# cr1m5onk1ng/text_similarity

Hardware: AMD Instinct MI355X
Metric: sentences/sec encoded + Mpairs/sec cosine top-k @ N=1M d=384 (higher is better)
Workload: dtype bf16 encoder / f16 selection / fp32 scores

## Files before the change

text_similarity_amd/csrc/encoder.hip:

```cpp
#include <math.h>
#include <cmath>

#include <stdlib.h>
#include <string.h>

#include <vector>

#include <type_traits>
#include <utility>

#include "common.h"
#include "gemm_pp.h"

namespace tsim {

__device__ __forceinline__ int64_t packed_off(int64_t t, int f, int W) {
    return ((t >> 5) * (W >> 3) + (f >> 3)) * 256 + (t & 31) * 8 + (f & 7);
}

template <int VPL, bool TYPED = false>
__global__ __launch_bounds__(256) void embed_ln_kernel(const int32_t *__restrict__ ids,
                                                       const int32_t *__restrict__ pos,
                                                       const float *__restrict__ word,
                                                       const float *__restrict__ pos_emb,
                                                       const float *__restrict__ type_tab,
                                                       const float *__restrict__ gamma,
                                                       const float *__restrict__ beta, float eps, int T, int H,
                                                       bf16_t *__restrict__ out, int vocab, int max_pos,
                                                       const int32_t *__restrict__ col, int max_len,
                                                       int *__restrict__ err_flags,
                                                       const int32_t *__restrict__ tok_type = nullptr, int n_types = 0) {
    const int lane = threadIdx.x & 63;
    const int t = blockIdx.x * 4 + (threadIdx.x >> 6);
    if (t >= T) return;
    int id = ids[t], ps = pos[t];
    int ty = 0;
    if constexpr (TYPED) ty = tok_type[t];
    int bad = 0;
    if (id < 0 || id >= vocab) { bad |= TSIM_ENC_ERR_TOKEN_ID; id = id < 0 ? 0 : vocab - 1; }
    if (ps < 0 || ps >= max_pos) { bad |= TSIM_ENC_ERR_POSITION; ps = ps < 0 ? 0 : max_pos - 1; }
    if (col[t] >= max_len || col[t] < 0) bad |= TSIM_ENC_ERR_MAX_LEN;
    if constexpr (TYPED) {
        if (ty < 0 || ty >= n_types) { bad |= TSIM_ENC_ERR_TOKEN_TYPE; ty = ty < 0 ? 0 : n_types - 1; }
    }
    if (bad && lane == 0) atomicOr(err_flags, bad);
    const float *w = word + (int64_t)id * H;
    const float *p = pos_emb + (int64_t)ps * H;
    const float *type_row = TYPED ? type_tab + (int64_t)ty * H : type_tab;
    float v[VPL], pv[VPL], tv[VPL];
#pragma unroll
    for (int i = 0; i < VPL; ++i) {
        v[i] = w[lane + i * 64];
        pv[i] = p[lane + i * 64];
    }
    if (type_row) {
#pragma unroll
        for (int i = 0; i < VPL; ++i) tv[i] = type_row[lane + i * 64];
    }
    float s = 0.f;
#pragma unroll
    for (int i = 0; i < VPL; ++i) {
        float a = v[i];
        if (type_row) a += tv[i];
        a += pv[i];
        v[i] = a;
        s += a;
    }
    const float mean = wave_sum(s) / (float)H;
    float q = 0.f;
#pragma unroll
    for (int i = 0; i < VPL; ++i) {
        const float dlt = v[i] - mean;
        q = fmaf(dlt, dlt, q);
    }
    const float rstd = 1.0f / sqrtf(wave_sum(q) / (float)H + eps);
#pragma unroll
    for (int i = 0; i < VPL; ++i) {
        const int j = lane + i * 64;
        out[(int64_t)t * H + j] = f32_to_bf16((v[i] - mean) * rstd * gamma[j] + beta[j]);
    }
}

enum { EPI_BIAS = 0, EPI_GELU = 1, EPI_RES_LN = 2 };

template <int BM, int BN, int BK, int WAVES_M, int WAVES_N, int NST = 2>
constexpr int gemm_lds_bytes() {
    return NST * (BM + BN) * BK * 2;
}

template <int BM, int BN, int BK, int WAVES_M, int WAVES_N, int EPI, int NST = 2>
__global__ __launch_bounds__(WAVES_M *WAVES_N * 64) void gemm_bf16_kernel(
    const bf16_t *__restrict__ X, const bf16_t *__restrict__ W, const float *__restrict__ bias,
    const bf16_t *__restrict__ res, const float *__restrict__ gamma, const float *__restrict__ beta, float eps,
    bf16_t *__restrict__ out, int M, int N, int K, int mtiles, int ntiles, const bf16_t *__restrict__ Wimg, int xpacked) {
    constexpr int NW = WAVES_M * WAVES_N;
    constexpr int TM = BM / WAVES_M, TN = BN / WAVES_N, MT = TM / 32, NT = TN / 32;
    constexpr int RB = BK * 2;
    constexpr int CPR = RB / 16;
    constexpr int RPS = 256 / RB;
    constexpr int X_BYTES = BM * RB, W_BYTES = BN * RB, STAGE = X_BYTES + W_BYTES;
    constexpr int PIECES = STAGE / 1024, XPIECES = X_BYTES / 1024;
    constexpr int KSTEPS = BK / 16;
    static_assert(TM % 32 == 0 && TN % 32 == 0 && X_BYTES % 1024 == 0 && W_BYTES % 1024 == 0, "tile shape");
    static_assert(NST == 2 || PIECES % NW == 0, "a deep ring needs equal DMA counts per wave");
    constexpr int PPW = (PIECES + NW - 1) / NW;
    extern __shared__ __attribute__((aligned(16))) char smem[];

    const int lane = threadIdx.x & 63;
    const int wave = __builtin_amdgcn_readfirstlane(threadIdx.x >> 6);
    const int wm = wave / WAVES_N, wn = wave % WAVES_N;
    const int r = lane & 31, h = lane >> 5;

    const int b = blockIdx.x, xcd = b & 7, jj = b >> 3;
    const int nt_id = jj % ntiles;
    const int mt_id = (jj / ntiles) * 8 + xcd;
    if (mt_id >= mtiles) return;
    const int m0 = mt_id * BM, n0 = nt_id * BN;

    constexpr int PPW_MAX = (PIECES + NW - 1) / NW;
    int src_off[PPW_MAX];
#pragma unroll
    for (int i = 0; i < PPW_MAX; ++i) {
        const int p = wave + i * NW;
        const bool isx = p < XPIECES;
        const int sl = (isx ? p : p - XPIECES) * 64 + lane;
        const int sr = sl >> 4, chp = sl & 15;
        const int ch = chp ^ (sr & 15);
        const int row = sr * RPS + ch / CPR, c = ch % CPR;
        src_off[i] = (isx && xpacked) ? (row >> 5) * K * 64 + (row & 31) * 16 + c * 512 : row * K * 2 + c * 16;
    }
    const int xkstride = xpacked ? (BK / 8) * 512 : BK * 2;
    const char *xbase = reinterpret_cast<const char *>(X + (int64_t)m0 * K);
    const char *wbase = reinterpret_cast<const char *>(W + (int64_t)n0 * K);
    const char *wimg = reinterpret_cast<const char *>(Wimg);
    auto piece_src = [&](int i, int p, int kt) __attribute__((always_inline)) -> const char * {
        if (p < XPIECES) return xbase + src_off[i] + kt * xkstride;
        if (wimg) return wimg + (int64_t)kt * W_BYTES + (p - XPIECES) * 1024 + lane * 16;
        return wbase + src_off[i] + kt * (BK * 2);
    };
    auto issue = [&](int kt, int stage) __attribute__((always_inline)) {
#pragma unroll
        for (int i = 0; i < PPW_MAX; ++i) {
            const int p = wave + i * NW;
            if (p < PIECES) glds16(piece_src(i, p, kt), smem + stage * STAGE + p * 1024);
        }
    };
    auto frag_off = [&](int row, int s) {
        const int sr = row / RPS;
        const int ch = (row % RPS) * CPR + 2 * s + h;
        return sr * 256 + ((ch ^ (sr & 15)) << 4);
    };

    f32x16 acc[NT][MT];
#pragma unroll
    for (int i = 0; i < NT; ++i)
#pragma unroll
        for (int gq = 0; gq < 4; ++gq) {
            const float4 bv = *reinterpret_cast<const float4 *>(bias + n0 + wn * TN + 4 * h + i * 32 + 8 * gq);
#pragma unroll
            for (int j = 0; j < MT; ++j) {
                acc[i][j][4 * gq + 0] = bv.x;
                acc[i][j][4 * gq + 1] = bv.y;
                acc[i][j][4 * gq + 2] = bv.z;
                acc[i][j][4 * gq + 3] = bv.w;
            }
        }
#if defined(TSIM_LN_DIAG) && TSIM_LN_DIAG == 3
    const int nk = 1;
#else
    const int nk = K / BK;
#endif
#pragma unroll
    for (int i = 0; i < NT; ++i)
#pragma unroll
        for (int j = 0; j < MT; ++j) asm volatile("" : "+v"(acc[i][j]));
    if constexpr (NST == 2) {
        issue(0, 0);
    } else {
#pragma unroll
        for (int i = 0; i < NST - 1; ++i) issue(i < nk ? i : nk - 1, i);
    }
    for (int kt = 0; kt < nk; ++kt) {
        const char *xs = smem + (kt % NST) * STAGE;
        const char *ws = xs + X_BYTES;
        auto load_frags = [&](int s, bf16x8 (&bx)[MT], bf16x8 (&aw)[NT]) __attribute__((always_inline)) {
#pragma unroll
            for (int j = 0; j < MT; ++j)
                bx[j] = *reinterpret_cast<const bf16x8 *>(xs + frag_off(wm * TM + j * 32 + r, s));
#pragma unroll
            for (int i = 0; i < NT; ++i)
                aw[i] = *reinterpret_cast<const bf16x8 *>(ws + frag_off(wn * TN + i * 32 + r, s));
        };
        if constexpr (NST == 2) {
            wait_vmcnt<0>();
            __builtin_amdgcn_s_barrier();
            bf16x8 bx[2][MT], aw[2][NT];
#if defined(TSIM_LN_DIAG) && (TSIM_LN_DIAG == 1 || TSIM_LN_DIAG == 4 || TSIM_LN_DIAG == 5)
            for (int s = 0; s < KSTEPS; ++s)
                if (kt + 1 < nk) {
#pragma unroll
                    for (int i = s * PPW_MAX / KSTEPS; i < (s + 1) * PPW_MAX / KSTEPS; ++i) {
                        const int p = wave + i * NW;
                        if (TSIM_LN_DIAG == 4 && p >= XPIECES) continue;
                        if (TSIM_LN_DIAG == 5 && p < XPIECES) continue;
                        if (p < PIECES) glds16(piece_src(i, p, kt + 1), smem + ((kt + 1) & 1) * STAGE + p * 1024);
                    }
                }
            continue;
#endif
            load_frags(0, bx[0], aw[0]);
#pragma unroll
            for (int s = 0; s < KSTEPS; ++s) {
                if (s + 1 < KSTEPS) load_frags(s + 1, bx[(s + 1) & 1], aw[(s + 1) & 1]);
#if defined(TSIM_LN_DIAG) && TSIM_LN_DIAG == 2
                if (false) {
#else
                if (kt + 1 < nk) {
#endif
#pragma unroll
                    for (int i = s * PPW_MAX / KSTEPS; i < (s + 1) * PPW_MAX / KSTEPS; ++i) {
                        const int p = wave + i * NW;
                        if (p < PIECES) glds16(piece_src(i, p, kt + 1), smem + ((kt + 1) & 1) * STAGE + p * 1024);
                    }
                }
#pragma unroll
                for (int i = 0; i < NT; ++i)
#pragma unroll
                    for (int j = 0; j < MT; ++j)
                        acc[i][j] = __builtin_amdgcn_mfma_f32_32x32x16_bf16(aw[s & 1][i], bx[s & 1][j], acc[i][j], 0, 0, 0);
            }
        } else {
            wait_vmcnt<(NST - 2) * PPW>();
            __builtin_amdgcn_s_barrier();
            const int nx = kt + NST - 1;
            issue(nx < nk ? nx : nk - 1, nx % NST);
#pragma unroll
            for (int s = 0; s < KSTEPS; ++s) {
                bf16x8 bx[MT], aw[NT];
                load_frags(s, bx, aw);
#pragma unroll
                for (int i = 0; i < NT; ++i)
#pragma unroll
                    for (int j = 0; j < MT; ++j)
                        acc[i][j] = __builtin_amdgcn_mfma_f32_32x32x16_bf16(aw[i], bx[j], acc[i][j], 0, 0, 0);
            }
        }
    }

    if constexpr (NST > 2) wait_vmcnt<0>();
    const int nbase = n0 + wn * TN + 4 * h;
    const int mbase = m0 + wm * TM + r;

    if constexpr (EPI == EPI_RES_LN) {
        float *red = reinterpret_cast<float *>(smem);
        __builtin_amdgcn_s_barrier();
#pragma unroll
        for (int j = 0; j < MT; ++j) {
            const int64_t m = m0 + wm * TM + j * 32 + r;
            const int64_t mr = m < M ? m : M - 1;
#pragma unroll
            for (int i = 0; i < NT; ++i)
#pragma unroll
                for (int gq = 0; gq < 4; gq += 2) {
                    const uint4 o = *reinterpret_cast<const uint4 *>(res + mr * N + n0 + wn * TN + i * 32 + 8 * gq + 8 * h);
                    auto s0 = __builtin_amdgcn_permlane32_swap(o.x, o.z, false, false);
                    auto s1 = __builtin_amdgcn_permlane32_swap(o.y, o.w, false, false);
                    const uint32_t a0 = s0[0], c0 = s0[1], a1 = s1[0], c1 = s1[1];
                    acc[i][j][4 * gq + 0] += __uint_as_float(a0 << 16);
                    acc[i][j][4 * gq + 1] += __uint_as_float(a0 & 0xffff0000u);
                    acc[i][j][4 * gq + 2] += __uint_as_float(a1 << 16);
                    acc[i][j][4 * gq + 3] += __uint_as_float(a1 & 0xffff0000u);
                    acc[i][j][4 * gq + 4] += __uint_as_float(c0 << 16);
                    acc[i][j][4 * gq + 5] += __uint_as_float(c0 & 0xffff0000u);
                    acc[i][j][4 * gq + 6] += __uint_as_float(c1 << 16);
                    acc[i][j][4 * gq + 7] += __uint_as_float(c1 & 0xffff0000u);
                }
        }
        float mean[MT], rstd[MT];
#pragma unroll
        for (int pass = 0; pass < 2; ++pass) {
#pragma unroll
            for (int j = 0; j < MT; ++j) {
                float s = 0.f;
#pragma unroll
                for (int i = 0; i < NT; ++i)
#pragma unroll
                    for (int g = 0; g < 16; ++g) {
                        if (pass == 0) {
                            s += acc[i][j][g];
                        } else {
                            const float dlt = acc[i][j][g] - mean[j];
                            s = fmaf(dlt, dlt, s);
                        }
                    }
                s += __shfl_xor(s, 32, 64);
                if (h == 0) red[(pass * WAVES_N + wn) * BM + wm * TM + j * 32 + r] = s;
            }
            __syncthreads();
#pragma unroll
            for (int j = 0; j < MT; ++j) {
                float s = 0.f;
#pragma unroll
                for (int w = 0; w < WAVES_N; ++w) s += red[(pass * WAVES_N + w) * BM + wm * TM + j * 32 + r];
                if (pass == 0)
                    mean[j] = s / (float)N;
                else
                    rstd[j] = 1.0f / sqrtf(s / (float)N + eps);
            }
        }
#pragma unroll
        for (int i = 0; i < NT; ++i) {
            float4 gv[4], be[4];
#pragma unroll
            for (int gq = 0; gq < 4; ++gq) {
                gv[gq] = *reinterpret_cast<const float4 *>(gamma + nbase + i * 32 + 8 * gq);
                be[gq] = *reinterpret_cast<const float4 *>(beta + nbase + i * 32 + 8 * gq);
            }
#pragma unroll
            for (int j = 0; j < MT; ++j) {
                uint32_t pk[8];
#pragma unroll
                for (int gq = 0; gq < 4; ++gq) {
                    const float y0 = fmaf((acc[i][j][4 * gq + 0] - mean[j]) * rstd[j], gv[gq].x, be[gq].x);
                    const float y1 = fmaf((acc[i][j][4 * gq + 1] - mean[j]) * rstd[j], gv[gq].y, be[gq].y);
                    const float y2 = fmaf((acc[i][j][4 * gq + 2] - mean[j]) * rstd[j], gv[gq].z, be[gq].z);
                    const float y3 = fmaf((acc[i][j][4 * gq + 3] - mean[j]) * rstd[j], gv[gq].w, be[gq].w);
                    pk[2 * gq] = pack_bf16x2(y0, y1);
                    pk[2 * gq + 1] = pack_bf16x2(y2, y3);
                }
                const int64_t m = m0 + wm * TM + j * 32 + r;
#pragma unroll
                for (int gq = 0; gq < 4; gq += 2) {
                    auto s0 = __builtin_amdgcn_permlane32_swap(pk[2 * gq], pk[2 * gq + 2], false, false);
                    auto s1 = __builtin_amdgcn_permlane32_swap(pk[2 * gq + 1], pk[2 * gq + 3], false, false);
                    if (m < M)
                        *reinterpret_cast<uint4 *>(out + m * N + n0 + wn * TN + i * 32 + 8 * gq + 8 * h) =
                            make_uint4(s0[0], s1[0], s0[1], s1[1]);
                }
            }
        }
    } else {
#pragma unroll
        for (int i = 0; i < NT; ++i)
#pragma unroll
            for (int gq = 0; gq < 4; ++gq) {
                const int n = nbase + i * 32 + 8 * gq;
#pragma unroll
                for (int j = 0; j < MT; ++j) {
                    const int64_t m = mbase + j * 32;
                    float y0 = acc[i][j][4 * gq + 0], y1 = acc[i][j][4 * gq + 1];
                    float y2 = acc[i][j][4 * gq + 2], y3 = acc[i][j][4 * gq + 3];
                    if constexpr (EPI == EPI_GELU) {
                        gelu2(y0, y1);
                        gelu2(y2, y3);
                    }
                    uint2 o;
                    o.x = pack_bf16x2(y0, y1);
                    o.y = pack_bf16x2(y2, y3);
                    *reinterpret_cast<uint2 *>(out + m * N + n) = o;
                }
            }
    }
}

constexpr int XR_BN = 192;
typedef __attribute__((ext_vector_type(4))) uint32_t u32x4;

#ifdef TSIM_PP_STAMPS
__device__ unsigned long long g_xr_stamps[8];
#define XR_T() __builtin_amdgcn_s_memtime()
#ifndef TSIM_XR_STAMP_TID
#define TSIM_XR_STAMP_TID 0
#endif
#define XR_ACC(i, v) do { if (threadIdx.x == TSIM_XR_STAMP_TID) atomicAdd(&g_xr_stamps[i], (unsigned long long)(v)); } while (0)
#else
#define XR_T() 0ull
#define XR_ACC(i, v) do { } while (0)
#endif

template <int... I, class Fn>
__device__ __forceinline__ void ff_static_for(std::integer_sequence<int, I...>, Fn &&f) {
    (f(std::integral_constant<int, I>{}), ...);
}

constexpr int X2_BN = 96, X2_BK = 128, X2_NSTAGE = 6, X2_PD = 4, X2_KG = 3, X2_NSUB = 3;

template <int EPI, bool PK>
__global__ __launch_bounds__(512) void gemm_xres2_kernel(const bf16_t *__restrict__ X, const bf16_t *__restrict__ W,
                                                         const float *__restrict__ bias, bf16_t *__restrict__ out,
                                                         int M, int N, int items_total) {
    constexpr int K = 384, KSTEPS = K / 16, NW = 8, BMX = NW * 32;
    constexpr int STAGE = X2_BN * X2_BK * 2;
    constexpr int PIECES = STAGE / 1024, PPW = PIECES / NW;
    static_assert(PIECES % NW == 0 && X2_KG * X2_BK == K, "tile shape");
    extern __shared__ __attribute__((aligned(16))) char smem[];
    const int lane = threadIdx.x & 63;
    const int wave = __builtin_amdgcn_readfirstlane(threadIdx.x >> 6);
    const int r = lane & 31, h = lane >> 5;
    const int ntiles = N / X2_BN;
    const int it0 = (int)((int64_t)items_total * blockIdx.x / gridDim.x);
    const int it1 = (int)((int64_t)items_total * (blockIdx.x + 1) / gridDim.x);
    const int total = (it1 - it0) * X2_KG;
    if (total <= 0) return;

    int src_off[PPW];
#pragma unroll
    for (int i = 0; i < PPW; ++i) {
        const int sl = (wave * PPW + i) * 64 + lane;
        const int row = sl >> 4, ch = (sl & 15) ^ (row & 15);
        src_off[i] = row * K * 2 + ch * 16;
    }
    auto issue_pieces = [&](int st, int stage, int i0, int i1) __attribute__((always_inline)) {
        const int s2 = st < total ? st : total - 1;
        const int j = (it0 + s2 / X2_KG) % ntiles, g = s2 % X2_KG;
        const char *base = reinterpret_cast<const char *>(W) + ((int64_t)j * X2_BN * K + g * X2_BK) * 2;
#if defined(TSIM_X2_DIAG) && (TSIM_X2_DIAG & 4)
        (void)base;
#else
        for (int i = i0; i < i1; ++i)
            glds16(base + src_off[i], smem + stage * STAGE + (wave * PPW + i) * 1024);
#endif
    };
    auto issue = [&](int st, int stage) __attribute__((always_inline)) { issue_pieces(st, stage, 0, PPW); };
    int cks[8];
#pragma unroll
    for (int ks = 0; ks < 8; ++ks) cks[ks] = r * 256 + (((2 * ks + h) ^ (r & 15)) << 4);

    const uint32_t bias_lds = (uint32_t)(uintptr_t)((__attribute__((address_space(3))) char *)smem) + X2_NSTAGE * STAGE;
    for (int p = wave; p * 256 < N; p += NW)
        if (p * 256 + lane * 4 < N) glds16(bias + p * 256 + lane * 4, smem + X2_NSTAGE * STAGE + p * 1024);
    wait_vmcnt<0>();
    __builtin_amdgcn_s_barrier();

    bf16x8 bx[KSTEPS];
    int cur_mb = -1, m0 = 0;
    f32x16 accA[X2_NSUB], accB[X2_NSUB];
    int old_m0 = 0, old_n0 = 0;
    int st = 0;
    int ring = 0;
    int young1 = 0, young2 = 0, young3 = 0;

    uint32_t old_rowoff = 0;
    const uint64_t out_base = (uint64_t)(uintptr_t)out;
    auto store_half = [&](const uint32_t (&pk)[8], int mrow0, int ncol, auto gqc) __attribute__((always_inline)) {
        constexpr int gq = decltype(gqc)::value;
        const bool full = mrow0 + 32 <= M;
        uint32_t a0 = pk[2 * gq], a1 = pk[2 * gq + 1], b0 = pk[2 * gq + 2], b1 = pk[2 * gq + 3];
        auto s0 = __builtin_amdgcn_permlane32_swap(a0, b0, false, false);
        auto s1 = __builtin_amdgcn_permlane32_swap(a1, b1, false, false);
        const u32x4 o = {s0[0], s1[0], s0[1], s1[1]};
        const uint32_t voff = old_rowoff + (uint32_t)(ncol + 8 * gq) * (PK ? 64u : 2u);
        const uint64_t ob = out_base;
#if !(defined(TSIM_X2_DIAG) && (TSIM_X2_DIAG & 1))
        if (full || mrow0 + r < M)
            asm volatile("global_store_dwordx4 %0, %1, %2\n\ts_nop 1" ::"v"(voff), "v"(o), "s"(ob) : "memory");
#else
        asm volatile("" ::"v"(voff), "v"(o));
#endif
    };
    auto finish2 = [&](float y0, float y1) __attribute__((always_inline)) -> uint32_t {
#if !(defined(TSIM_X2_DIAG) && (TSIM_X2_DIAG & 2))
        if constexpr (EPI == EPI_GELU) gelu2(y0, y1);
#endif
        return pack_bf16x2(y0, y1);
    };

#pragma unroll
    for (int i = 0; i < X2_PD; ++i) issue(i, i);
    [[maybe_unused]] unsigned x2_n = 0, x2_w = 0, x2_c = 0, x2_e = 0;
    auto run_item = [&](f32x16 (&cur)[X2_NSUB], f32x16 (&old)[X2_NSUB], int item, auto with_old) __attribute__((always_inline)) {
        constexpr bool OLD = decltype(with_old)::value;
        if (item / ntiles != cur_mb) {
            cur_mb = item / ntiles;
            m0 = cur_mb * BMX + wave * 32;
            const bf16_t *xp = X + (int64_t)(m0 + r) * K + 8 * h;
#pragma unroll
            for (int s = 0; s < KSTEPS; ++s) bx[s] = *reinterpret_cast<const bf16x8 *>(xp + 16 * s);
#pragma unroll
            for (int s = 0; s < KSTEPS; ++s) asm volatile("" : "+v"(bx[s]));
            young1 = young2 = young3 = 0;
        }
        const int n0 = (item % ntiles) * X2_BN;
        const uint32_t baddr = bias_lds + (n0 + 4 * h) * 4;
        ff_static_for(std::make_integer_sequence<int, X2_NSUB>{}, [&](auto ic) __attribute__((always_inline)) {
            constexpr int i = decltype(ic)::value;
            f32x4 bv[4];
            asm volatile("ds_read_b128 %0, %1 offset:%2" : "=v"(bv[0]) : "v"(baddr), "n"((i * 32 + 0) * 4) : "memory");
            asm volatile("ds_read_b128 %0, %1 offset:%2" : "=v"(bv[1]) : "v"(baddr), "n"((i * 32 + 8) * 4) : "memory");
            asm volatile("ds_read_b128 %0, %1 offset:%2" : "=v"(bv[2]) : "v"(baddr), "n"((i * 32 + 16) * 4) : "memory");
            asm volatile("ds_read_b128 %0, %1 offset:%2" : "=v"(bv[3]) : "v"(baddr), "n"((i * 32 + 24) * 4) : "memory");
            asm volatile("s_waitcnt lgkmcnt(0)" : "+v"(bv[0]), "+v"(bv[1]), "+v"(bv[2]), "+v"(bv[3])::"memory");
#pragma unroll
            for (int q = 0; q < 16; ++q) cur[i][q] = bv[q >> 2][q & 3];
        });
#pragma unroll
        for (int g = 0; g < X2_KG; ++g) {
            asm volatile("" : "+s"(ring));
            const int stage = ring;
            [[maybe_unused]] const unsigned long long xs0 = XR_T();
            if ((st & 1) == 0) {
                const int ys = (young1 >= 0 && young2 >= 0 && young3 >= 0) ? young1 + young2 + young3 : 0;
                if (ys == 6) wait_vmcnt<2 * PPW + 6>();
                else if (ys == 4) wait_vmcnt<2 * PPW + 4>();
                else if (ys == 2) wait_vmcnt<2 * PPW + 2>();
                else wait_vmcnt<2 * PPW>();
                __builtin_amdgcn_s_barrier();
            }
            __builtin_amdgcn_sched_barrier(0);
            [[maybe_unused]] const unsigned long long xs1 = XR_T();
            static_assert(PPW == 3, "issue schedule below places three pieces");
            uint32_t pk[8];
            {
                constexpr int PF = 3, NRD = 8 * X2_NSUB;
                lds_u32x4 fr[PF + 1];
                const uint32_t wsl = (uint32_t)(uintptr_t)((__attribute__((address_space(3))) char *)smem) + stage * STAGE;
                auto rd = [&](auto nc) __attribute__((always_inline)) {
                    constexpr int n = decltype(nc)::value;
                    lds_read_b128_imm<(n % X2_NSUB) * 8192>(fr[n % (PF + 1)], wsl + cks[n / X2_NSUB]);
                };
                ff_static_for(std::make_integer_sequence<int, PF>{}, rd);
                ff_static_for(std::make_integer_sequence<int, NRD>{}, [&](auto nc) __attribute__((always_inline)) {
                    constexpr int n = decltype(nc)::value;
                    constexpr int ks = n / X2_NSUB, i = n % X2_NSUB;
                    if constexpr (n + PF < NRD) rd(std::integral_constant<int, n + PF>{});
                    constexpr int younger = n + PF < NRD ? PF : NRD - 1 - n;
                    lgkm_wait_counted<younger>(fr[n % (PF + 1)]);
                    cur[i] = __builtin_amdgcn_mfma_f32_32x32x16_bf16(__builtin_bit_cast(bf16x8, fr[n % (PF + 1)]), bx[g * 8 + ks], cur[i], 0, 0, 0);
                    if constexpr (i == X2_NSUB - 1) {
                        if constexpr (ks == 1 || ks == 3 || ks == 5)
                            issue_pieces(st + X2_PD, (stage + X2_PD) % X2_NSTAGE, ks >> 1, (ks >> 1) + 1);
                        if constexpr (OLD) pk[ks] = finish2(old[g][2 * ks], old[g][2 * ks + 1]);
                    }
                });
            }
#ifdef TSIM_PP_STAMPS
#pragma unroll
            for (int i = 0; i < X2_NSUB; ++i) asm volatile("" : "+v"(cur[i]));
#endif
            [[maybe_unused]] const unsigned long long xs2 = XR_T();
            young3 = young2;
            young2 = young1;
            young1 = 0;
            if constexpr (OLD) {
                store_half(pk, old_m0, old_n0 + g * 32, std::integral_constant<int, 0>{});
                store_half(pk, old_m0, old_n0 + g * 32, std::integral_constant<int, 2>{});
#if defined(TSIM_X2_DIAG) && (TSIM_X2_DIAG & 1)
                young1 = 0;
#else
                young1 = old_m0 + 32 <= M ? 2 : -1;
#endif
            }
            ++st;
            ring = ring + 1 == X2_NSTAGE ? 0 : ring + 1;
#ifdef TSIM_PP_STAMPS
            { const unsigned long long xs3 = XR_T(); x2_n += 1; x2_w += (unsigned)(xs1 - xs0); x2_c += (unsigned)(xs2 - xs1); x2_e += (unsigned)(xs3 - xs2); }
#endif
        }
        old_m0 = m0;
        old_n0 = n0;
        old_rowoff = PK ? (uint32_t)(m0 >> 5) * (uint32_t)(N * 64) + 16u * r + 512u * h
                        : (uint32_t)(m0 + r) * (uint32_t)(N * 2) + 16u * h;
    };
    int item = it0;
    run_item(accA, accB, item++, std::false_type{});
    for (; item + 2 <= it1; item += 2) {
        run_item(accB, accA, item, std::true_type{});
        run_item(accA, accB, item + 1, std::true_type{});
    }
    const bool lastA = item >= it1;
    if (!lastA) run_item(accB, accA, item, std::true_type{});
    wait_vmcnt<0>();
    auto flush = [&](f32x16 (&acc)[X2_NSUB]) __attribute__((always_inline)) {
#pragma unroll
        for (int g = 0; g < X2_NSUB; ++g) {
            uint32_t pk[8];
#pragma unroll
            for (int ks = 0; ks < 8; ++ks) pk[ks] = finish2(acc[g][2 * ks], acc[g][2 * ks + 1]);
            store_half(pk, old_m0, old_n0 + g * 32, std::integral_constant<int, 0>{});
            store_half(pk, old_m0, old_n0 + g * 32, std::integral_constant<int, 2>{});
        }
    };
    if (lastA) flush(accA); else flush(accB);
    XR_ACC(0, x2_n); XR_ACC(1, x2_w); XR_ACC(3, x2_c); XR_ACC(4, x2_e); XR_ACC(6, x2_n / 3);
}

__global__ __launch_bounds__(256) void pack_gemm_w_kernel(const uint4 *__restrict__ W, uint4 *__restrict__ img, int BN, int BK, int K) {
    const int slots = BN * BK * 2 / 16;
    const int64_t u = (int64_t)blockIdx.x * 256 + threadIdx.x;
    if (u >= (int64_t)slots * (K / BK)) return;
    const int kt = (int)(u / slots), sl = (int)(u % slots);
    const int cpr = BK * 2 / 16, rps = 256 / (BK * 2);
    const int sr = sl >> 4, ch = (sl & 15) ^ (sr & 15);
    const int row = sr * rps + ch / cpr, c = ch % cpr;
    img[u] = W[((int64_t)row * K + (int64_t)kt * BK) * 2 / 16 + c];
}
__global__ __launch_bounds__(256) void pack_frag_w_kernel(const uint4 *__restrict__ W, uint4 *__restrict__ img, int N, int K) {
    const int64_t u = (int64_t)blockIdx.x * 256 + threadIdx.x;
    if (u >= (int64_t)N * K / 8) return;
    const int lane = (int)(u & 63), blk = (int)(u >> 6);
    const int nt = N / 32, s = blk / nt, j = blk % nt, r = lane & 31, h = lane >> 5;
    img[u] = W[((int64_t)(32 * j + r) * K + 16 * s + 8 * h) / 8];
}
constexpr int LR_BK = 32, LR_WBYTES = 384 * LR_BK * 2;

template <int NW, int LR_NST>
__global__ __launch_bounds__(NW * 64) void ln_rows_gemm_kernel(const bf16_t *__restrict__ X, const bf16_t *__restrict__ Wimg,
                                                               const float *__restrict__ bias, const bf16_t *__restrict__ res,
                                                               const float *__restrict__ gamma, const float *__restrict__ beta,
                                                               float eps, bf16_t *__restrict__ out, int M, int K, int xpacked) {
    constexpr int N = 384, XBYTES = NW * 32 * LR_BK * 2, STAGE = XBYTES + LR_WBYTES;
    constexpr int XP = XBYTES / 1024, PIECES = STAGE / 1024, PPW = PIECES / NW;
    static_assert(PIECES % NW == 0 && XP == 2 * NW, "every wave issues two X pieces and PPW - 2 W pieces per k-tile");
    extern __shared__ __attribute__((aligned(16))) char smem[];
    const int lane = threadIdx.x & 63;
    const int wave = __builtin_amdgcn_readfirstlane(threadIdx.x >> 6);
    const int r = lane & 31, h = lane >> 5;
    const int m0 = blockIdx.x * (NW * 32);
    const int nk = K / LR_BK;

    f32x16 acc[12];
#pragma unroll
    for (int t = 0; t < 12; ++t)
#pragma unroll
        for (int gq = 0; gq < 4; ++gq) {
            const f32x4 bv = *reinterpret_cast<const f32x4 *>(bias + 32 * t + 8 * gq + 4 * h);
#pragma unroll
            for (int e = 0; e < 4; ++e) acc[t][4 * gq + e] = bv[e];
        }
    const char *xsrc[2];
#pragma unroll
    for (int i = 0; i < 2; ++i) {
        const int sl = (wave + i * NW) * 64 + lane;
        const int sr = sl >> 4, ch = (sl & 15) ^ (sr & 15);
        const int row = sr * 4 + (ch >> 2);
        const int64_t m = m0 + row < M ? m0 + row : M - 1;
        xsrc[i] = xpacked ? reinterpret_cast<const char *>(X + packed_off(m, (ch & 3) * 8, K))
                          : reinterpret_cast<const char *>(X) + m * K * 2 + (ch & 3) * 16;
    }
    const int xkstride = xpacked ? (LR_BK / 8) * 512 : LR_BK * 2;
    const char *wsrc = reinterpret_cast<const char *>(Wimg) + lane * 16;
    auto issue = [&](int kt, int stage) __attribute__((always_inline)) {
        const int k2 = kt < nk ? kt : nk - 1;
        char *dst = smem + stage * STAGE;
#pragma unroll
        for (int i = 0; i < 2; ++i) glds16(xsrc[i] + k2 * xkstride, dst + (wave + i * NW) * 1024);
#pragma unroll
        for (int i = 2; i < PPW; ++i)
            glds16(wsrc + (int64_t)k2 * LR_WBYTES + (wave + i * NW - XP) * 1024, dst + (wave + i * NW) * 1024);
    };
    const uint32_t lbase = (uint32_t)(uintptr_t)((__attribute__((address_space(3))) char *)smem);
    uint32_t xo[2];
#pragma unroll
    for (int sk = 0; sk < 2; ++sk) {
        const int ch = (r & 3) * 4 + 2 * sk + h;
        xo[sk] = lbase + wave * 2048 + (r >> 2) * 256 + ((ch ^ ((((wave & 1) << 3) + (r >> 2)) & 15)) << 4);
    }
    const uint32_t wl = lbase + XBYTES + lane * 16;

    static_assert(LR_NST >= 3 && (LR_NST - 2) * PPW <= 63, "ring depth");
#pragma unroll
    for (int i = 0; i < LR_NST - 1; ++i) issue(i, i);
#pragma unroll
    for (int t = 0; t < 12; ++t) asm volatile("" : "+v"(acc[t]));
    auto do_tile = [&](int kt, auto stc) __attribute__((always_inline)) {
        constexpr int stage = decltype(stc)::value;
        wait_vmcnt<(LR_NST - 2) * PPW>();
        __builtin_amdgcn_s_barrier();
        issue(kt + LR_NST - 1, (stage + LR_NST - 1) % LR_NST);
        constexpr int PF = 4, NRD = 24;
        lds_u32x4 bfr[2], fr[PF + 1];
        const uint32_t so = stage * STAGE;
        lds_read_b128_imm<0>(bfr[0], xo[0] + so);
        lds_read_b128_imm<0>(bfr[1], xo[1] + so);
        const uint32_t wa = wl + so;
        auto rd = [&](auto nc) __attribute__((always_inline)) {
            constexpr int n = decltype(nc)::value;
            lds_read_b128_imm<n * 1024>(fr[n % (PF + 1)], wa);
        };
        ff_static_for(std::make_integer_sequence<int, PF>{}, rd);
        ff_static_for(std::make_integer_sequence<int, NRD>{}, [&](auto nc) __attribute__((always_inline)) {
            constexpr int n = decltype(nc)::value;
            if constexpr (n + PF < NRD) rd(std::integral_constant<int, n + PF>{});
            constexpr int younger = n + PF < NRD ? PF : NRD - 1 - n;
            lgkm_wait_counted<younger>(fr[n % (PF + 1)]);
            if constexpr (n == 0) { asm volatile("" : "+v"(bfr[0])); asm volatile("" : "+v"(bfr[1])); }
            acc[n % 12] = __builtin_amdgcn_mfma_f32_32x32x16_bf16(__builtin_bit_cast(bf16x8, fr[n % (PF + 1)]),
                                                                   __builtin_bit_cast(bf16x8, bfr[n / 12]), acc[n % 12], 0, 0, 0);
        });
    };
    int kt = 0;
    for (; kt + LR_NST <= nk; kt += LR_NST)
        ff_static_for(std::make_integer_sequence<int, LR_NST>{}, [&](auto sc) __attribute__((always_inline)) {
            do_tile(kt + decltype(sc)::value, sc);
        });
    ff_static_for(std::make_integer_sequence<int, LR_NST - 1>{}, [&](auto sc) __attribute__((always_inline)) {
        if (kt + decltype(sc)::value < nk) do_tile(kt + decltype(sc)::value, sc);
    });
    wait_vmcnt<0>();

    const int64_t m = m0 + wave * 32 + r;
    const bool live = m < M;
    const int64_t mr = live ? m : M - 1;
#pragma unroll
    for (int t = 0; t < 12; ++t)
#pragma unroll
        for (int gq = 0; gq < 4; gq += 2) {
            const uint4 o = *reinterpret_cast<const uint4 *>(res + mr * N + 32 * t + 8 * gq + 8 * h);
            auto s0 = __builtin_amdgcn_permlane32_swap(o.x, o.z, false, false);
            auto s1 = __builtin_amdgcn_permlane32_swap(o.y, o.w, false, false);
            const uint32_t a0 = s0[0], c0 = s0[1], a1 = s1[0], c1 = s1[1];
            acc[t][4 * gq + 0] += __uint_as_float(a0 << 16);
            acc[t][4 * gq + 1] += __uint_as_float(a0 & 0xffff0000u);
            acc[t][4 * gq + 2] += __uint_as_float(a1 << 16);
            acc[t][4 * gq + 3] += __uint_as_float(a1 & 0xffff0000u);
            acc[t][4 * gq + 4] += __uint_as_float(c0 << 16);
            acc[t][4 * gq + 5] += __uint_as_float(c0 & 0xffff0000u);
            acc[t][4 * gq + 6] += __uint_as_float(c1 << 16);
            acc[t][4 * gq + 7] += __uint_as_float(c1 & 0xffff0000u);
        }
    float mean, rstd;
#pragma unroll
    for (int pass = 0; pass < 2; ++pass) {
        float tot = 0.f;
#pragma unroll
        for (int w = 0; w < 4; ++w) {
            float sg = 0.f;
#pragma unroll
            for (int t = 3 * w; t < 3 * w + 3; ++t)
#pragma unroll
                for (int q = 0; q < 16; ++q) {
                    if (pass == 0) {
                        sg += acc[t][q];
                    } else {
                        const float dlt = acc[t][q] - mean;
                        sg = fmaf(dlt, dlt, sg);
                    }
                }
            sg += __shfl_xor(sg, 32, 64);
            tot += sg;
        }
        if (pass == 0)
            mean = tot / (float)N;
        else
            rstd = 1.0f / sqrtf(tot / (float)N + eps);
    }
#pragma unroll
    for (int t = 0; t < 12; ++t) {
        uint32_t pk[8];
#pragma unroll
        for (int gq = 0; gq < 4; ++gq) {
            const int n = 32 * t + 8 * gq + 4 * h;
            const f32x4 gv = *reinterpret_cast<const f32x4 *>(gamma + n), bv = *reinterpret_cast<const f32x4 *>(beta + n);
            const float o0 = fmaf((acc[t][4 * gq + 0] - mean) * rstd, gv[0], bv[0]);
            const float o1 = fmaf((acc[t][4 * gq + 1] - mean) * rstd, gv[1], bv[1]);
            const float o2 = fmaf((acc[t][4 * gq + 2] - mean) * rstd, gv[2], bv[2]);
            const float o3 = fmaf((acc[t][4 * gq + 3] - mean) * rstd, gv[3], bv[3]);
            pk[2 * gq] = pack_bf16x2(o0, o1);
            pk[2 * gq + 1] = pack_bf16x2(o2, o3);
        }
#pragma unroll
        for (int gq = 0; gq < 4; gq += 2) {
            auto s0 = __builtin_amdgcn_permlane32_swap(pk[2 * gq], pk[2 * gq + 2], false, false);
            auto s1w = __builtin_amdgcn_permlane32_swap(pk[2 * gq + 1], pk[2 * gq + 3], false, false);
            if (live) *reinterpret_cast<uint4 *>(out + m * N + 32 * t + 8 * gq + 8 * h) = make_uint4(s0[0], s1w[0], s0[1], s1w[1]);
        }
    }
}

template <int DH, bool REL, bool PK = false>
__global__ __launch_bounds__(256) __attribute__((amdgpu_waves_per_eu(DH <= 32 ? 6 : 4))) void attention_kernel(const bf16_t *__restrict__ qkv,
                                                        const int32_t *__restrict__ cu, const int32_t *__restrict__ col,
                                                        const float *__restrict__ relb, int relw, int H,
                                                        int heads, float scale, bf16_t *__restrict__ ctx, int B, int xcd_map) {
    constexpr int KS = DH / 16;
    constexpr int OT = (DH + 31) / 32;
    constexpr int ROWB = DH * 2 < 64 ? 64 : DH * 2;
    __shared__ __attribute__((aligned(16))) char vimg[4 * 32 * ROWB];
    typedef __attribute__((ext_vector_type(4))) short s16x4;
    const int lane = threadIdx.x & 63;
    const int wave = __builtin_amdgcn_readfirstlane(threadIdx.x >> 6);
    int seq = blockIdx.x;
    if (xcd_map) {
        seq = (blockIdx.x & 7) * (gridDim.x >> 3) + (blockIdx.x >> 3);
        if (seq >= B) return;
    }
    const int head = blockIdx.y * 4 + wave, qb = blockIdx.z;
    const int t0 = cu[seq], S = cu[seq + 1] - t0;
    if (qb * 32 >= S || head >= heads) return;
    const int r = lane & 31, h = lane >> 5;
    const int64_t H3 = 3 * (int64_t)H;
    const int qi = qb * 32 + r;
    const int tq = t0 + (qi < S ? qi : S - 1);

    bf16x8 qf[KS];
    {
        const bf16_t *qp = PK ? qkv + packed_off(tq, head * DH + 8 * h, (int)H3) : qkv + tq * H3 + head * DH + 8 * h;
#pragma unroll
        for (int s = 0; s < KS; ++s) {
            qf[s] = *reinterpret_cast<const bf16x8 *>(qp + (PK ? 2 * 256 : 16) * s);
        }
    }
    const int qcol = REL ? col[tq] : 0;
    f32x16 o[OT];
#pragma unroll
    for (int ob = 0; ob < OT; ++ob)
#pragma unroll
        for (int g = 0; g < 16; ++g) o[ob][g] = 0.f;
    float m = -INFINITY, l = 0.f;

    for (int k0 = 0; k0 < S; k0 += 32) {
        const int kr = k0 + r;
        const int tk = t0 + (kr < S ? kr : S - 1);
        f32x16 sc;
#pragma unroll
        for (int g = 0; g < 16; ++g) sc[g] = 0.f;
        constexpr int CH = DH / 16;
        uint4 vr[CH];
        {
            const bf16_t *kp = PK ? qkv + packed_off(tk, H + head * DH + 8 * h, (int)H3) : qkv + tk * H3 + H + head * DH + 8 * h;
            const bf16_t *vsrc = PK ? qkv + packed_off(tk, 2 * H + head * DH + h * (DH / 2), (int)H3)
                                    : qkv + tk * H3 + 2 * H + head * DH + h * (DH / 2);
            bf16x8 kf[KS];
#pragma unroll
            for (int s = 0; s < KS; ++s) kf[s] = *reinterpret_cast<const bf16x8 *>(kp + (PK ? 2 * 256 : 16) * s);
#pragma unroll
            for (int c = 0; c < CH; ++c) vr[c] = *reinterpret_cast<const uint4 *>(vsrc + (PK ? 256 : 8) * c);
#pragma unroll
            for (int s = 0; s < KS; ++s) sc = __builtin_amdgcn_mfma_f32_32x32x16_bf16(kf[s], qf[s], sc, 0, 0, 0);
        }
        float bm = -INFINITY;
#pragma unroll
        for (int g = 0; g < 16; ++g) {
            const int key = k0 + (g & 3) + 8 * (g >> 2) + 4 * h;
            float v = sc[g] * scale;
            if (REL) {
                const int kc = col[t0 + (key < S ? key : S - 1)];
                v += relb[head * relw + (kc - qcol) + (relw >> 1)];
            }
            v = key < S ? v : -INFINITY;
            sc[g] = v;
            bm = fmaxf(bm, v);
        }
        bm = fmaxf(bm, __shfl_xor(bm, 32, 64));
        const float mn = fmaxf(m, bm);
        const float corr = __expf(m - mn);
        float ps = 0.f;
#pragma unroll
        for (int g = 0; g < 16; ++g) {
            sc[g] = __expf(sc[g] - mn);
            ps += sc[g];
        }
        ps += __shfl_xor(ps, 32, 64);
        l = l * corr + ps;
        m = mn;
#pragma unroll
        for (int ob = 0; ob < OT; ++ob)
#pragma unroll
            for (int g = 0; g < 16; ++g) o[ob][g] *= corr;
        bf16x8 pf[2];
#pragma unroll
        for (int s = 0; s < 2; ++s)
#pragma unroll
            for (int j = 0; j < 8; ++j) pf[s][j] = (__bf16)sc[8 * s + j];
        {
            char *vrow = vimg + wave * (32 * ROWB) + r * ROWB + h * DH;
#pragma unroll
            for (int c = 0; c < CH; ++c) *reinterpret_cast<uint4 *>(vrow + 16 * c) = vr[c];
        }
        __builtin_amdgcn_wave_barrier();
#pragma unroll
        for (int ob = 0; ob < OT; ++ob) {
            const bool iv = ob * 32 + r < DH;
            const int grp16 = (lane >> 4) & 1, q4 = (lane & 15) >> 2, p4 = lane & 3;
#pragma unroll
            for (int s = 0; s < 2; ++s) {
                bf16x8 vf;
#pragma unroll
                for (int half = 0; half < 2; ++half) {
                    const int key = 16 * s + 8 * half + 4 * h + q4;
                    const char *ad = vimg + wave * (32 * ROWB) + key * ROWB + (ob * 32 + grp16 * 16 + 4 * p4) * 2;
                    const s16x4 t = __builtin_amdgcn_ds_read_tr16_b64_v4i16((__attribute__((address_space(3))) s16x4 *)ad);
#pragma unroll
                    for (int e = 0; e < 4; ++e)
                        vf[4 * half + e] = __builtin_bit_cast(__bf16, (bf16_t)(iv ? (bf16_t)t[e] : (bf16_t)0));
                }
                o[ob] = __builtin_amdgcn_mfma_f32_32x32x16_bf16(vf, pf[s], o[ob], 0, 0, 0);
            }
        }
        __builtin_amdgcn_wave_barrier();
    }
    if (qi < S) {
        const float inv = 1.0f / l;
        bf16_t *op = ctx + (int64_t)(t0 + qi) * H + head * DH + 4 * h;
#pragma unroll
        for (int ob = 0; ob < OT; ++ob)
#pragma unroll
            for (int gq = 0; gq < 4; ++gq) {
                const int i = ob * 32 + 8 * gq;
                if (i + 4 * h < DH) {
                    uint2 w;
                    w.x = pack_bf16x2(o[ob][4 * gq] * inv, o[ob][4 * gq + 1] * inv);
                    w.y = pack_bf16x2(o[ob][4 * gq + 2] * inv, o[ob][4 * gq + 3] * inv);
                    *reinterpret_cast<uint2 *>(op + i) = w;
                }
            }
    }
}

template <int NP, int MODE = TSIM_POOL_MEAN, bool NORM = false>
__global__ __launch_bounds__(256) void pool_packed_kernel(const bf16_t *__restrict__ x,
                                                          const int32_t *__restrict__ cu, int B, int H,
                                                          float *__restrict__ pooled, unit_t *__restrict__ unit,
                                                          int ld_unit, float *__restrict__ rho_max) {
    __shared__ __attribute__((aligned(16))) float rows[4][NP * 512];
    const int lane = threadIdx.x & 63, w = threadIdx.x >> 6;
    const int b = blockIdx.x * 4 + w;
    if (b >= B) return;
    const int t0 = cu[b], t1 = cu[b + 1];
    float s[NP][8];
#pragma unroll
    for (int p = 0; p < NP; ++p)
#pragma unroll
        for (int e = 0; e < 8; ++e) s[p][e] = MODE == TSIM_POOL_MAX ? -INFINITY : 0.f;
    auto add_row = [&](int p, const uint4 &v) __attribute__((always_inline)) {
        const uint32_t wv[4] = {v.x, v.y, v.z, v.w};
#pragma unroll
        for (int q = 0; q < 4; ++q) {
            s[p][2 * q] += __uint_as_float(wv[q] << 16);
            s[p][2 * q + 1] += __uint_as_float(wv[q] & 0xffff0000u);
        }
    };
    if constexpr (MODE == TSIM_POOL_CLS) {
#pragma unroll
        for (int p = 0; p < NP; ++p) {
            const int f0 = (lane + 64 * p) * 8;
            if (f0 >= H || t1 <= t0) continue;
            const uint4 v = *reinterpret_cast<const uint4 *>(x + (int64_t)t0 * H + f0);
            const uint32_t wv[4] = {v.x, v.y, v.z, v.w};
#pragma unroll
            for (int q = 0; q < 4; ++q) {
                s[p][2 * q] = __uint_as_float(wv[q] << 16);
                s[p][2 * q + 1] = __uint_as_float(wv[q] & 0xffff0000u);
            }
        }
    } else if constexpr (MODE == TSIM_POOL_MAX) {
#pragma unroll
        for (int p = 0; p < NP; ++p) {
            const int f0 = (lane + 64 * p) * 8;
            if (f0 >= H) continue;
            const bf16_t *xp = x + f0;
            for (int t = t0; t < t1; t += 8) {
                uint4 v[8];
#pragma unroll
                for (int u = 0; u < 8; ++u) v[u] = *reinterpret_cast<const uint4 *>(xp + (int64_t)(t + u < t1 ? t + u : t1 - 1) * H);
#pragma unroll
                for (int u = 0; u < 8; ++u) {
                    const uint32_t wv[4] = {v[u].x, v[u].y, v[u].z, v[u].w};
#pragma unroll
                    for (int q = 0; q < 4; ++q) {
                        s[p][2 * q] = fmaxf(s[p][2 * q], __uint_as_float(wv[q] << 16));
                        s[p][2 * q + 1] = fmaxf(s[p][2 * q + 1], __uint_as_float(wv[q] & 0xffff0000u));
                    }
                }
            }
        }
    } else {
#pragma unroll
        for (int p = 0; p < NP; ++p) {
            const int f0 = (lane + 64 * p) * 8;
            if (f0 >= H) continue;
            const bf16_t *xp = x + f0;
            for (int t = t0; t < t1; t += 8) {
                uint4 v[8];
#pragma unroll
                for (int u = 0; u < 8; ++u) v[u] = *reinterpret_cast<const uint4 *>(xp + (int64_t)(t + u < t1 ? t + u : t1 - 1) * H);
#pragma unroll
                for (int u = 0; u < 8; ++u) {
                    if (t + u >= t1) v[u] = make_uint4(0u, 0u, 0u, 0u);
                    add_row(p, v[u]);
                }
            }
        }
    }
    const float den = MODE == TSIM_POOL_MEAN_SQRT_LEN ? sqrtf(fmaxf((float)(t1 - t0), 1e-9f)) : fmaxf((float)(t1 - t0), 1e-9f);
#pragma unroll
    for (int p = 0; p < NP; ++p) {
        const int f0 = (lane + 64 * p) * 8;
#pragma unroll
        for (int e = 0; e < 8; ++e) {
            if constexpr (MODE == TSIM_POOL_MEAN || MODE == TSIM_POOL_MEAN_SQRT_LEN) s[p][e] = s[p][e] / den;
            else if constexpr (MODE == TSIM_POOL_MAX) s[p][e] = t1 > t0 ? s[p][e] : 0.f;
        }
        if (f0 < H) {
            const float4 lo = make_float4(s[p][0], s[p][1], s[p][2], s[p][3]), hi = make_float4(s[p][4], s[p][5], s[p][6], s[p][7]);
            if (!NORM && pooled) {
                *reinterpret_cast<float4 *>(pooled + (int64_t)b * H + f0) = lo;
                *reinterpret_cast<float4 *>(pooled + (int64_t)b * H + f0 + 4) = hi;
            }
            *reinterpret_cast<float4 *>(&rows[w][f0]) = lo;
            *reinterpret_cast<float4 *>(&rows[w][f0 + 4]) = hi;
        }
    }
    if constexpr (NORM) {
        __builtin_amdgcn_wave_barrier();
        double ss = 0.0;
        for (int jx = lane; jx < H; jx += 64) {
            const float v = rows[w][jx];
            ss = fma((double)v, (double)v, ss);
        }
        const double inv = canonical_inv_norm(ss, 1e-12f);
#pragma unroll
        for (int p = 0; p < NP; ++p) {
            const int f0 = (lane + 64 * p) * 8;
#pragma unroll
            for (int e = 0; e < 8; ++e) s[p][e] = canonical_scale_f32(s[p][e], inv);
            if (f0 < H) {
                const float4 lo = make_float4(s[p][0], s[p][1], s[p][2], s[p][3]), hi = make_float4(s[p][4], s[p][5], s[p][6], s[p][7]);
                if (pooled) {
                    *reinterpret_cast<float4 *>(pooled + (int64_t)b * H + f0) = lo;
                    *reinterpret_cast<float4 *>(pooled + (int64_t)b * H + f0 + 4) = hi;
                }
                *reinterpret_cast<float4 *>(&rows[w][f0]) = lo;
                *reinterpret_cast<float4 *>(&rows[w][f0 + 4]) = hi;
            }
        }
    }
    if (unit) {
        __builtin_amdgcn_wave_barrier();
        double ss = 0.0;
        for (int jx = lane; jx < H; jx += 64) {
            const float v = rows[w][jx];
            ss = fma((double)v, (double)v, ss);
        }
        const double inv = canonical_inv_norm(ss, 1e-8f);
        double r2 = 0.0;
#pragma unroll
        for (int p = 0; p < NP; ++p) {
            const int f0 = (lane + 64 * p) * 8;
            if (f0 < H) {
                f16x8 u;
#pragma unroll
                for (int e = 0; e < 8; ++e) {
                    u[e] = canonical_unit_elem(s[p][e], inv);
                    const double de = (double)(float)u[e] - (double)s[p][e] * inv;
                    r2 = fma(de, de, r2);
                }
                *reinterpret_cast<f16x8 *>(unit + (int64_t)b * ld_unit + f0) = u;
            }
        }
        for (int jx = H + lane; jx < ld_unit; jx += 64) unit[(int64_t)b * ld_unit + jx] = 0;
        if (rho_max) {
            const float rho = rho_round_up(sqrt(wave_sum_f64(r2)));
            if (lane == 0) rho_publish(rho_max, rho);
        }
    }
}

constexpr int CLS_ROWS = 8;
constexpr int CLS_MAX_H = 768;
constexpr int CLS_WIDE_H = 1024;
constexpr int CLS_MAX_LABELS = 32;

__global__ __launch_bounds__(CLS_MAX_H) void cls_head_kernel(const bf16_t *__restrict__ x, const int32_t *__restrict__ cu,
                                                             int B, int H, const float *__restrict__ wpT,
                                                             const float *__restrict__ bp, const float *__restrict__ wc,
                                                             const float *__restrict__ bc, int n_labels,
                                                             float *__restrict__ logits) {
    __shared__ __attribute__((aligned(16))) float xs[CLS_MAX_H][CLS_ROWS];
    __shared__ float ps[CLS_ROWS][CLS_MAX_H];
    const int j = threadIdx.x;
    const int b0 = blockIdx.x * CLS_ROWS;
#pragma unroll
    for (int r = 0; r < CLS_ROWS; ++r) {
        const int b = b0 + r;
        float v = 0.f;
        if (b < B) {
            const int t0 = cu[b];
            if (cu[b + 1] > t0) v = bf16_to_f32(x[(int64_t)t0 * H + j]);
        }
        xs[j][r] = v;
    }
    __syncthreads();
    float acc[CLS_ROWS];
#pragma unroll
    for (int r = 0; r < CLS_ROWS; ++r) acc[r] = 0.f;
    for (int k0 = 0; k0 < H; k0 += 8) {
        float w[8];
#pragma unroll
        for (int u = 0; u < 8; ++u) w[u] = wpT[(int64_t)(k0 + u) * H + j];
#pragma unroll
        for (int u = 0; u < 8; ++u) {
            const float4 lo = *reinterpret_cast<const float4 *>(&xs[k0 + u][0]);
            const float4 hi = *reinterpret_cast<const float4 *>(&xs[k0 + u][4]);
            const float xv[CLS_ROWS] = {lo.x, lo.y, lo.z, lo.w, hi.x, hi.y, hi.z, hi.w};
#pragma unroll
            for (int r = 0; r < CLS_ROWS; ++r) acc[r] = fmaf(w[u], xv[r], acc[r]);
        }
    }
    const float bj = bp[j];
#pragma unroll
    for (int r = 0; r < CLS_ROWS; ++r) ps[r][j] = tanhf(acc[r] + bj);
    __syncthreads();
    const int lane = j & 63, wave = j >> 6, n_waves = H >> 6;
    const int n_out = CLS_ROWS * n_labels;
    for (int o = wave; o < n_out; o += n_waves) {
        const int r = o / n_labels, c = o - r * n_labels;
        const int b = b0 + r;
        if (b >= B) break;
        float s = 0.f;
        for (int i = lane; i < H; i += 64) s = fmaf(wc[(int64_t)c * H + i], ps[r][i], s);
        s = wave_sum(s);
        if (lane == 0) logits[(int64_t)b * n_labels + c] = s + bc[c];
    }
}

template <int MAXH, int ACT>
__global__ __launch_bounds__(MAXH) void cls_head_wide_kernel(const bf16_t *__restrict__ x, const int32_t *__restrict__ cu,
                                                             int B, int H, const float *__restrict__ wpT,
                                                             const float *__restrict__ bp, const float *__restrict__ wc,
                                                             const float *__restrict__ bc, int n_labels,
                                                             float *__restrict__ logits) {
    __shared__ __attribute__((aligned(16))) float xs[MAXH][CLS_ROWS];
    __shared__ float ps[CLS_ROWS][MAXH];
    const int j = threadIdx.x;
    const int b0 = blockIdx.x * CLS_ROWS;
#pragma unroll
    for (int r = 0; r < CLS_ROWS; ++r) {
        const int b = b0 + r;
        float v = 0.f;
        if (b < B) {
            const int t0 = cu[b];
            if (cu[b + 1] > t0) v = bf16_to_f32(x[(int64_t)t0 * H + j]);
        }
        xs[j][r] = v;
    }
    __syncthreads();
    float acc[CLS_ROWS];
#pragma unroll
    for (int r = 0; r < CLS_ROWS; ++r) acc[r] = 0.f;
    for (int k0 = 0; k0 < H; k0 += 8) {
        float w[8];
#pragma unroll
        for (int u = 0; u < 8; ++u) w[u] = wpT[(int64_t)(k0 + u) * H + j];
#pragma unroll
        for (int u = 0; u < 8; ++u) {
            const float4 lo = *reinterpret_cast<const float4 *>(&xs[k0 + u][0]);
            const float4 hi = *reinterpret_cast<const float4 *>(&xs[k0 + u][4]);
            const float xv[CLS_ROWS] = {lo.x, lo.y, lo.z, lo.w, hi.x, hi.y, hi.z, hi.w};
#pragma unroll
            for (int r = 0; r < CLS_ROWS; ++r) acc[r] = fmaf(w[u], xv[r], acc[r]);
        }
    }
    const float bj = bp[j];
#pragma unroll
    for (int r = 0; r < CLS_ROWS; ++r) ps[r][j] = ACT == TSIM_ACT_RELU ? fmaxf(acc[r] + bj, 0.f) : tanhf(acc[r] + bj);
    __syncthreads();
    const int lane = j & 63, wave = j >> 6, n_waves = H >> 6;
    const int n_out = CLS_ROWS * n_labels;
    for (int o = wave; o < n_out; o += n_waves) {
        const int r = o / n_labels, c = o - r * n_labels;
        const int b = b0 + r;
        if (b >= B) break;
        float s = 0.f;
        for (int i = lane; i < H; i += 64) s = fmaf(wc[(int64_t)c * H + i], ps[r][i], s);
        s = wave_sum(s);
        if (lane == 0) logits[(int64_t)b * n_labels + c] = s + bc[c];
    }
}

constexpr int DN_ROWS = 16;
constexpr int DN_MAX = 1024;
constexpr int DN_WAVES = 8;

__device__ __forceinline__ float4 load4_or_zero(const float *p, bool ok) {
    float4 v = make_float4(0.f, 0.f, 0.f, 0.f);
    if (ok) v = *reinterpret_cast<const float4 *>(p);
    return v;
}

template <int NT>
__global__ __launch_bounds__(64 * DN_WAVES) void dense_rows_kernel(const float *__restrict__ x, int B, int d_in, const float *__restrict__ wt,
                                                         const float *__restrict__ bias, int d_out, int act, int normalize,
                                                         float *__restrict__ out, unit_t *__restrict__ unit, int ld_unit,
                                                         float *__restrict__ rho_max) {
    extern __shared__ __attribute__((aligned(16))) float ys[];
    const int lane = threadIdx.x & 63, wv = threadIdx.x >> 6;
    const int r0 = blockIdx.x * DN_ROWS;
    if (wt) {
        const int i = lane & 15, g = lane >> 4;
        const int ntt = (d_out + 15) >> 4;
        const float *xp = x + (int64_t)min(r0 + i, B - 1) * d_in + 4 * g;
        const float *wp[NT];
#pragma unroll
        for (int t = 0; t < NT; ++t) wp[t] = wt + (int64_t)min((wv + DN_WAVES * t) * 16 + i, d_out - 1) * d_in + 4 * g;
        f32x4 acc[NT];
#pragma unroll
        for (int t = 0; t < NT; ++t) acc[t] = f32x4{0.f, 0.f, 0.f, 0.f};
        float4 a = load4_or_zero(xp, 4 * g < d_in), bw[NT];
#pragma unroll
        for (int t = 0; t < NT; ++t) bw[t] = load4_or_zero(wp[t], wv + DN_WAVES * t < ntt && 4 * g < d_in);
        for (int k0 = 0; k0 < d_in; k0 += 16) {
            const int k1 = k0 + 16;
            const bool kin = k1 + 4 * g < d_in;
            const float4 an = load4_or_zero(xp + k1, kin);
            float4 bn[NT];
#pragma unroll
            for (int t = 0; t < NT; ++t) bn[t] = load4_or_zero(wp[t] + k1, wv + DN_WAVES * t < ntt && kin);
#pragma unroll
            for (int t = 0; t < NT; ++t) {
                if (wv + DN_WAVES * t < ntt) {
                    acc[t] = __builtin_amdgcn_mfma_f32_16x16x4f32(a.x, bw[t].x, acc[t], 0, 0, 0);
                    acc[t] = __builtin_amdgcn_mfma_f32_16x16x4f32(a.y, bw[t].y, acc[t], 0, 0, 0);
                    acc[t] = __builtin_amdgcn_mfma_f32_16x16x4f32(a.z, bw[t].z, acc[t], 0, 0, 0);
                    acc[t] = __builtin_amdgcn_mfma_f32_16x16x4f32(a.w, bw[t].w, acc[t], 0, 0, 0);
                }
            }
            a = an;
#pragma unroll
            for (int t = 0; t < NT; ++t) bw[t] = bn[t];
        }
#pragma unroll
        for (int t = 0; t < NT; ++t) {
            const int col = (wv + DN_WAVES * t) * 16 + i;
            if (col < d_out) {
#pragma unroll
                for (int r = 0; r < 4; ++r) ys[(4 * g + r) * d_out + col] = acc[t][r];
            }
        }
    } else {
        for (int k = threadIdx.x; k < DN_ROWS * d_out; k += 64 * DN_WAVES) {
            const int r = k / d_out;
            ys[k] = r0 + r < B ? x[(int64_t)(r0 + r) * d_in + (k - r * d_out)] : 0.f;
        }
    }
    __syncthreads();
    for (int r = wv; r < DN_ROWS; r += DN_WAVES) {
        const int b = r0 + r;
        if (b >= B) break;
        float *y = ys + r * d_out;
        for (int j = lane; j < d_out; j += 64) {
            float v = y[j];
            if (bias) v += bias[j];
            if (act == TSIM_ACT_TANH) v = tanhf(v);
            y[j] = v;
        }
        if (normalize) {
            double ss = 0.0;
            for (int j = lane; j < d_out; j += 64) ss = fma((double)y[j], (double)y[j], ss);
            const double inv = canonical_inv_norm(ss, 1e-12f);
            for (int j = lane; j < d_out; j += 64) y[j] = canonical_scale_f32(y[j], inv);
        }
        if (out)
            for (int j = lane; j < d_out; j += 64) out[(int64_t)b * d_out + j] = y[j];
        if (unit) {
            double ss = 0.0;
            for (int j = lane; j < d_out; j += 64) ss = fma((double)y[j], (double)y[j], ss);
            const double inv = canonical_inv_norm(ss, 1e-8f);
            double r2 = 0.0;
            for (int j = lane; j < ld_unit; j += 64) {
                unit_t hv = (unit_t)0;
                if (j < d_out) {
                    hv = canonical_unit_elem(y[j], inv);
                    const double de = (double)(float)hv - (double)y[j] * inv;
                    r2 = fma(de, de, r2);
                }
                unit[(int64_t)b * ld_unit + j] = hv;
            }
            if (rho_max) {
                const float rho = rho_round_up(sqrt(wave_sum_f64(r2)));
                if (lane == 0) rho_publish(rho_max, rho);
            }
        }
    }
}

static int dense_rows_launch(const float *x, int B, int d_in, const float *w, const float *bias, int d_out, int act, int normalize,
                             float *out, unit_t *unit, int ld_unit, float *rho_max, hipStream_t st) {
    if (B <= 0) return TSIM_OK;
    const dim3 grid((unsigned)((B + DN_ROWS - 1) / DN_ROWS));
    const size_t lds = (size_t)DN_ROWS * d_out * sizeof(float);
#define DENSE(NT) hipLaunchKernelGGL(dense_rows_kernel<NT>, grid, dim3(64 * DN_WAVES), lds, st, x, B, d_in, w, bias, d_out, act, normalize, out, unit, ld_unit, rho_max)
    const int nt = ((d_out + 15) / 16 + DN_WAVES - 1) / DN_WAVES;
    if (nt <= 1) DENSE(1); else if (nt <= 2) DENSE(2); else if (nt <= 3) DENSE(3); else if (nt <= 4) DENSE(4);
    else if (nt <= 6) DENSE(6); else DENSE(8);
#undef DENSE
    TSIM_HIP_CHECK(hipGetLastError());
    return TSIM_OK;
}

static int dense_check(int d_in, int d_out, int act, const float *w) {
    TSIM_REQUIRE(d_in >= 8 && d_in <= DN_MAX && d_in % 8 == 0, "dense: d_in=%d outside [8, %d] or not a multiple of 8", d_in, DN_MAX);
    TSIM_REQUIRE(d_out >= 8 && d_out <= DN_MAX && d_out % 8 == 0, "dense: d_out=%d outside [8, %d] or not a multiple of 8", d_out,
                 DN_MAX);
    TSIM_REQUIRE(w || d_out == d_in, "dense: without a weight matrix d_out (%d) must equal d_in (%d)", d_out, d_in);
    TSIM_REQUIRE(act == TSIM_ACT_IDENTITY || act == TSIM_ACT_TANH, "dense: unknown activation %d (TSIM_ACT_IDENTITY, TSIM_ACT_TANH)",
                 act);
    TSIM_REQUIRE(((uintptr_t)w & 15) == 0, "dense: the weight matrix must be 16-byte aligned");
    return TSIM_OK;
}

static uint16_t host_f32_to_bf16(float f) {
    uint32_t u;
    memcpy(&u, &f, 4);
    if ((u & 0x7fffffffu) > 0x7f800000u) return (uint16_t)((u >> 16) | 0x40);
    u += 0x7fffu + ((u >> 16) & 1u);
    return (uint16_t)(u >> 16);
}

struct DevBuf {
    void *p = nullptr;
    ~DevBuf() {
        if (p) (void)hipFree(p);
    }
};

}

using namespace tsim;

struct tsim_encoder {
    tsim_encoder_config cfg;
    int Tp = 0;
    float *word = nullptr, *pos = nullptr, *type0 = nullptr, *emb_g = nullptr, *emb_b = nullptr, *relb = nullptr;
    int relw = 0;
    int n_types = 0;
    float *head_wpT = nullptr, *head_bp = nullptr, *head_wc = nullptr, *head_bc = nullptr;
    int n_labels = 0;
    int head_act = TSIM_ACT_TANH;
    struct Layer {
        bf16_t *wqkv, *wo, *w1, *w2;
        bf16_t *pqkv = nullptr, *po = nullptr;
        bf16_t *lo = nullptr, *l2 = nullptr;
        bf16_t *lo32 = nullptr, *l232 = nullptr;
        uint8_t *qqkv = nullptr, *qo = nullptr, *q1 = nullptr, *q2 = nullptr;
        uint8_t *sqkv = nullptr, *so = nullptr, *s1 = nullptr, *s2 = nullptr;
        float *bqkv, *bo, *b1, *b2, *g1, *be1, *g2, *be2;
    };
    std::vector<Layer> layers;
    std::vector<void *> allocs;
    bf16_t *x0 = nullptr, *x1 = nullptr, *qkv = nullptr, *ctx = nullptr, *h1 = nullptr;
    float *ybuf = nullptr;
    float *lnimg = nullptr;
    float *head_x = nullptr;
    uint8_t *aq = nullptr, *as = nullptr, *hq = nullptr, *hs = nullptr;
    int *err_flags = nullptr;
};

namespace tsim {

static int dev_alloc(tsim_encoder *e, size_t bytes, void **out) {
    void *p = nullptr;
    hipError_t err = hipMalloc(&p, bytes);
    if (err != hipSuccess) return fail(TSIM_ENOMEM, "hipMalloc(%zu) failed: %s", bytes, hipGetErrorString(err));
    e->allocs.push_back(p);
    *out = p;
    return TSIM_OK;
}

static int upload_f32(tsim_encoder *e, const float *h, size_t n, float **out) {
    int rc = dev_alloc(e, n * 4, (void **)out);
    if (rc) return rc;
    TSIM_HIP_CHECK(hipMemcpy(*out, h, n * 4, hipMemcpyHostToDevice));
    return TSIM_OK;
}

static int upload_bf16(tsim_encoder *e, const std::vector<const float *> &parts, size_t n_each, bf16_t **out) {
    std::vector<uint16_t> tmp(n_each * parts.size());
    for (size_t p = 0; p < parts.size(); ++p)
        for (size_t i = 0; i < n_each; ++i) tmp[p * n_each + i] = host_f32_to_bf16(parts[p][i]);
    int rc = dev_alloc(e, tmp.size() * 2, (void **)out);
    if (rc) return rc;
    TSIM_HIP_CHECK(hipMemcpy(*out, tmp.data(), tmp.size() * 2, hipMemcpyHostToDevice));
    return TSIM_OK;
}

static uint8_t host_f32_to_e4m3(float v) {
    const uint8_t sign = std::signbit(v) ? 0x80 : 0;
    const double a = std::fabs((double)v);
    if (a == 0.0) return sign;
    int exp;
    const double mant = std::frexp(a, &exp);
    long byte;
    if (a >= std::ldexp(1.0, -6))
        byte = ((long)(exp - 1 + 7) << 3) + std::lrint((mant * 2.0 - 1.0) * 8.0);
    else
        byte = std::lrint(std::ldexp(a, 9));
    if (byte > 0x7e) byte = 0x7e;
    return (uint8_t)byte | sign;
}

static int upload_mxfp8(tsim_encoder *e, const std::vector<const float *> &parts, size_t n_rows, size_t K, uint8_t **q,
                        uint8_t **sc) {
    const size_t rows = n_rows * parts.size(), nb = K / 32;
    std::vector<uint8_t> hq(rows * K), hs(rows * nb);
    for (size_t p = 0; p < parts.size(); ++p)
        for (size_t r = 0; r < n_rows; ++r)
            for (size_t b = 0; b < nb; ++b) {
                const float *src = parts[p] + r * K + b * 32;
                float amax = 0.f;
                for (int i = 0; i < 32; ++i) amax = std::fmax(amax, std::fabs(src[i]));
                int sexp = 0;
                if (amax > 0.f) {
                    int ex;
                    (void)std::frexp((double)amax, &ex);
                    sexp = ex - 1 - 8;
                    sexp = sexp < -127 ? -127 : (sexp > 127 ? 127 : sexp);
                }
                uint8_t *dst = hq.data() + (p * n_rows + r) * K + b * 32;
                for (int i = 0; i < 32; ++i) {
                    double y = std::ldexp((double)src[i], -sexp);
                    y = y > 448.0 ? 448.0 : (y < -448.0 ? -448.0 : y);
                    dst[i] = host_f32_to_e4m3((float)y);
                }
                hs[(p * n_rows + r) * nb + b] = (uint8_t)(sexp + 127);
            }
    int rc = dev_alloc(e, hq.size(), (void **)q);
    if (rc) return rc;
    if ((rc = dev_alloc(e, hs.size(), (void **)sc))) return rc;
    TSIM_HIP_CHECK(hipMemcpy(*q, hq.data(), hq.size(), hipMemcpyHostToDevice));
    TSIM_HIP_CHECK(hipMemcpy(*sc, hs.data(), hs.size(), hipMemcpyHostToDevice));
    return TSIM_OK;
}

static int mpnet_bucket(int rel, int num_buckets) {
    int ret = 0;
    int n = -rel;
    const int nb = num_buckets / 2;
    if (n < 0) {
        ret += nb;
        n = -n;
    }
    const int max_exact = nb / 2;
    if (n < max_exact) return ret + n;
    const float v = logf((float)n / (float)max_exact) / (float)log(128.0 / max_exact) * (float)(nb - max_exact);
    int large = max_exact + (int)v;
    if (large > nb - 1) large = nb - 1;
    return ret + large;
}

template <int BM, int BN, int BK, int WM, int WN, int EPI, int NST = 2>
static int launch_gemm(const bf16_t *X, const bf16_t *W, const float *bias, const bf16_t *res, const float *gamma,
                       const float *beta, float eps, bf16_t *out, int M, int N, int K, hipStream_t st,
                       const bf16_t *Wimg = nullptr, bool xpacked = false) {
    constexpr int lds = gemm_lds_bytes<BM, BN, BK, WM, WN, NST>();
    static_assert(lds <= 160 * 1024, "LDS budget");
    auto kern = gemm_bf16_kernel<BM, BN, BK, WM, WN, EPI, NST>;
    static DevOnce lds_once;
    TSIM_MAX_LDS(lds_once, kern, lds);
    if (N % BN != 0 || K % BK != 0) return fail(TSIM_EUNSUPPORTED, "gemm: N=%d K=%d not tileable by %dx%d", N, K, BN, BK);
    const int mtiles = (M + BM - 1) / BM, ntiles = N / BN;
    const int grid = ((mtiles + 7) / 8) * 8 * ntiles;
    if (Wimg && ntiles != 1) return fail(TSIM_EINVAL, "gemm: a packed W image needs BN == N");
    hipLaunchKernelGGL(kern, dim3(grid), dim3(WM * WN * 64), lds, st, X, W, bias, res, gamma, beta, eps, out, M, N, K,
                       mtiles, ntiles, Wimg, xpacked ? 1 : 0);
    TSIM_HIP_CHECK(hipGetLastError());
    return TSIM_OK;
}

template <int EPI, bool PK>
static int gemm_xres2(const bf16_t *X, const bf16_t *W, const float *bias, bf16_t *out, int M, int N, hipStream_t st) {
    constexpr int lds = X2_NSTAGE * X2_BN * X2_BK * 2 + 8192;
    if (N > 2048) return fail(TSIM_EUNSUPPORTED, "gemm_xres2: N=%d > 2048", N);
    if (((int64_t)M + 256) * N * 2 >= (1ll << 32)) return fail(TSIM_EUNSUPPORTED, "gemm_xres2: output of %d x %d exceeds 4 GiB", M, N);
    auto kern = gemm_xres2_kernel<EPI, PK>;
    static DevOnce lds_once;
    TSIM_MAX_LDS(lds_once, kern, lds);
    const int items = ((M + 255) / 256) * (N / X2_BN);
    const int grid = items < 256 ? items : 256;
    hipLaunchKernelGGL(kern, dim3(grid), dim3(512), lds, st, X, W, bias, out, M, N, items);
    TSIM_HIP_CHECK(hipGetLastError());
    return TSIM_OK;
}

typedef __attribute__((ext_vector_type(4))) uint32_t lt_u32x4;
constexpr int LT_PF = 12;

template <int PF>
__device__ __forceinline__ void lt_gemm_slice(const bf16_t *__restrict__ X, const bf16_t *__restrict__ Wimg32,
                                              const float *__restrict__ bias, const bf16_t *__restrict__ res, int M, int K,
                                              int xpacked, int wn, int m0, f32x16 (&acc)[3]) {
    constexpr int N = 384, NT = 3;
    const int lane = threadIdx.x & 63;
    const int r = lane & 31, h = lane >> 5;
    const int ksteps = K / 16;

    const int64_t mrow = (int64_t)(m0 + r < M ? m0 + r : M - 1);
    const char *xp = reinterpret_cast<const char *>(X) +
                     (xpacked ? (int64_t)(m0 >> 5) * K * 64 + h * 512 + r * 16
                              : (mrow * K + 8 * h) * 2);
    const int xstep = xpacked ? 1024 : 32;
    const char *wp = reinterpret_cast<const char *>(Wimg32) + (int64_t)(NT * wn) * 1024 + lane * 16;
    constexpr int WSTEP = (N / 32) * 1024;

#pragma unroll
    for (int i = 0; i < NT; ++i)
#pragma unroll
        for (int gq = 0; gq < 4; ++gq) {
            const float4 bv = *reinterpret_cast<const float4 *>(bias + wn * 96 + 4 * h + i * 32 + 8 * gq);
            acc[i][4 * gq + 0] = bv.x;
            acc[i][4 * gq + 1] = bv.y;
            acc[i][4 * gq + 2] = bv.z;
            acc[i][4 * gq + 3] = bv.w;
        }
#pragma unroll
    for (int i = 0; i < NT; ++i) asm volatile("" : "+v"(acc[i]));

    lt_u32x4 fw[PF][NT], fx[PF];
    auto issue = [&](auto slotc, int s) __attribute__((always_inline)) {
        constexpr int slot = decltype(slotc)::value;
        const int sc = s < ksteps ? s : ksteps - 1;
        const char *w = wp + (int64_t)sc * WSTEP;
        const char *x = xp + (int64_t)sc * xstep;
        lt_u32x4 &f0 = fw[slot][0], &f1 = fw[slot][1], &f2 = fw[slot][2], &f3 = fx[slot];
        asm volatile("global_load_dwordx4 %0, %1, off" : "=v"(f0) : "v"(w) : "memory");
        asm volatile("global_load_dwordx4 %0, %1, off offset:1024" : "=v"(f1) : "v"(w) : "memory");
        asm volatile("global_load_dwordx4 %0, %1, off offset:2048" : "=v"(f2) : "v"(w) : "memory");
        asm volatile("global_load_dwordx4 %0, %1, off" : "=v"(f3) : "v"(x) : "memory");
    };
    ff_static_for(std::make_integer_sequence<int, PF>{}, [&](auto sc) __attribute__((always_inline)) { issue(sc, decltype(sc)::value); });
    for (int s0 = 0; s0 < ksteps; s0 += PF) {
        ff_static_for(std::make_integer_sequence<int, PF>{}, [&](auto sc) __attribute__((always_inline)) {
            constexpr int slot = decltype(sc)::value;
            lt_u32x4 &f0 = fw[slot][0], &f1 = fw[slot][1], &f2 = fw[slot][2], &f3 = fx[slot];
            asm volatile("s_waitcnt vmcnt(%4)" : "+v"(f0), "+v"(f1), "+v"(f2), "+v"(f3) : "n"(4 * (PF - 1)) : "memory");
            const bf16x8 bx = __builtin_bit_cast(bf16x8, f3);
            acc[0] = __builtin_amdgcn_mfma_f32_32x32x16_bf16(__builtin_bit_cast(bf16x8, f0), bx, acc[0], 0, 0, 0);
            acc[1] = __builtin_amdgcn_mfma_f32_32x32x16_bf16(__builtin_bit_cast(bf16x8, f1), bx, acc[1], 0, 0, 0);
            acc[2] = __builtin_amdgcn_mfma_f32_32x32x16_bf16(__builtin_bit_cast(bf16x8, f2), bx, acc[2], 0, 0, 0);
            asm volatile("" : "+v"(f0), "+v"(f1), "+v"(f2), "+v"(f3));
            issue(sc, s0 + slot + PF);
        });
    }
    wait_vmcnt<0>();

    {
        const int64_t m = m0 + r;
        const int64_t mr = m < M ? m : M - 1;
#pragma unroll
        for (int i = 0; i < NT; ++i)
#pragma unroll
            for (int gq = 0; gq < 4; gq += 2) {
                const uint4 o = *reinterpret_cast<const uint4 *>(res + mr * N + wn * 96 + i * 32 + 8 * gq + 8 * h);
                auto s0 = __builtin_amdgcn_permlane32_swap(o.x, o.z, false, false);
                auto s1 = __builtin_amdgcn_permlane32_swap(o.y, o.w, false, false);
                const uint32_t a0 = s0[0], c0 = s0[1], a1 = s1[0], c1 = s1[1];
                acc[i][4 * gq + 0] += __uint_as_float(a0 << 16);
                acc[i][4 * gq + 1] += __uint_as_float(a0 & 0xffff0000u);
                acc[i][4 * gq + 2] += __uint_as_float(a1 << 16);
                acc[i][4 * gq + 3] += __uint_as_float(a1 & 0xffff0000u);
                acc[i][4 * gq + 4] += __uint_as_float(c0 << 16);
                acc[i][4 * gq + 5] += __uint_as_float(c0 & 0xffff0000u);
                acc[i][4 * gq + 6] += __uint_as_float(c1 << 16);
                acc[i][4 * gq + 7] += __uint_as_float(c1 & 0xffff0000u);
            }
    }
}

__device__ __forceinline__ void lt_layernorm(f32x16 (&acc)[3], float *red, const float *__restrict__ gamma,
                                             const float *__restrict__ beta, float eps, bf16_t *__restrict__ out, int M, int wn,
                                             int m0) {
    constexpr int N = 384, NT = 3, WAVES_N = 4, BM = 32;
    const int lane = threadIdx.x & 63;
    const int r = lane & 31, h = lane >> 5;
    const int nbase = wn * 96 + 4 * h;
    float mean = 0.f, rstd = 0.f;
#pragma unroll
    for (int pass = 0; pass < 2; ++pass) {
        float s = 0.f;
#pragma unroll
        for (int i = 0; i < NT; ++i)
#pragma unroll
            for (int g = 0; g < 16; ++g) {
                if (pass == 0) {
                    s += acc[i][g];
                } else {
                    const float dlt = acc[i][g] - mean;
                    s = fmaf(dlt, dlt, s);
                }
            }
        s += __shfl_xor(s, 32, 64);
        if (h == 0) red[(pass * WAVES_N + wn) * BM + r] = s;
        __syncthreads();
        float t = 0.f;
#pragma unroll
        for (int w = 0; w < WAVES_N; ++w) t += red[(pass * WAVES_N + w) * BM + r];
        if (pass == 0)
            mean = t / (float)N;
        else
            rstd = 1.0f / sqrtf(t / (float)N + eps);
    }
#pragma unroll
    for (int i = 0; i < NT; ++i) {
        float4 gv[4], be[4];
#pragma unroll
        for (int gq = 0; gq < 4; ++gq) {
            gv[gq] = *reinterpret_cast<const float4 *>(gamma + nbase + i * 32 + 8 * gq);
            be[gq] = *reinterpret_cast<const float4 *>(beta + nbase + i * 32 + 8 * gq);
        }
        uint32_t pk[8];
#pragma unroll
        for (int gq = 0; gq < 4; ++gq) {
            const float y0 = fmaf((acc[i][4 * gq + 0] - mean) * rstd, gv[gq].x, be[gq].x);
            const float y1 = fmaf((acc[i][4 * gq + 1] - mean) * rstd, gv[gq].y, be[gq].y);
            const float y2 = fmaf((acc[i][4 * gq + 2] - mean) * rstd, gv[gq].z, be[gq].z);
            const float y3 = fmaf((acc[i][4 * gq + 3] - mean) * rstd, gv[gq].w, be[gq].w);
            pk[2 * gq] = pack_bf16x2(y0, y1);
            pk[2 * gq + 1] = pack_bf16x2(y2, y3);
        }
        const int64_t m = m0 + r;
#pragma unroll
        for (int gq = 0; gq < 4; gq += 2) {
            auto s0 = __builtin_amdgcn_permlane32_swap(pk[2 * gq], pk[2 * gq + 2], false, false);
            auto s1 = __builtin_amdgcn_permlane32_swap(pk[2 * gq + 1], pk[2 * gq + 3], false, false);
            if (m < M)
                *reinterpret_cast<uint4 *>(out + m * N + wn * 96 + i * 32 + 8 * gq + 8 * h) = make_uint4(s0[0], s1[0], s0[1], s1[1]);
        }
    }
}

template <int PF>
__global__ __launch_bounds__(256) __attribute__((amdgpu_waves_per_eu(1, 1))) void ln_tail_gemm_kernel(
    const bf16_t *__restrict__ X, const bf16_t *__restrict__ Wimg32, const float *__restrict__ bias, const bf16_t *__restrict__ res,
    const float *__restrict__ gamma, const float *__restrict__ beta, float eps, bf16_t *__restrict__ out, int M, int K, int xpacked) {
    __shared__ float red[2 * 4 * 32];
    const int wn = __builtin_amdgcn_readfirstlane(threadIdx.x >> 6);
    const int m0 = blockIdx.x * 32;
    f32x16 acc[3];
    lt_gemm_slice<PF>(X, Wimg32, bias, res, M, K, xpacked, wn, m0, acc);
    lt_layernorm(acc, red, gamma, beta, eps, out, M, wn, m0);
}

constexpr int LS_MAX_BLOCKS = 256;

template <int PF, int S>
__global__ __launch_bounds__(256 / S) __attribute__((amdgpu_waves_per_eu(1, 1))) void ln_split_gemm_kernel(
    const bf16_t *__restrict__ X, const bf16_t *__restrict__ Wimg32, const float *__restrict__ bias, const bf16_t *__restrict__ res,
    float4 *__restrict__ img, int M, int K, int xpacked) {
    const int blk = blockIdx.x / S, sl = blockIdx.x % S;
    const int wn = __builtin_amdgcn_readfirstlane(sl * (4 / S) + (threadIdx.x >> 6));
    const int m0 = blk * 32;
    f32x16 acc[3];
    lt_gemm_slice<PF>(X, Wimg32, bias, res, M, K, xpacked, wn, m0, acc);
    float4 *dst = img + (int64_t)(blk * 4 + wn) * 12 * 64 + (threadIdx.x & 63);
#pragma unroll
    for (int i = 0; i < 3; ++i)
#pragma unroll
        for (int gq = 0; gq < 4; ++gq)
            dst[(i * 4 + gq) * 64] = make_float4(acc[i][4 * gq + 0], acc[i][4 * gq + 1], acc[i][4 * gq + 2], acc[i][4 * gq + 3]);
}

__global__ __launch_bounds__(256) void ln_split_finish_kernel(const float4 *__restrict__ img, const float *__restrict__ gamma,
                                                              const float *__restrict__ beta, float eps, bf16_t *__restrict__ out,
                                                              int M) {
    __shared__ float red[2 * 4 * 32];
    const int wn = __builtin_amdgcn_readfirstlane(threadIdx.x >> 6);
    const int m0 = blockIdx.x * 32;
    const float4 *src = img + (int64_t)(blockIdx.x * 4 + wn) * 12 * 64 + (threadIdx.x & 63);
    f32x16 acc[3];
#pragma unroll
    for (int i = 0; i < 3; ++i)
#pragma unroll
        for (int gq = 0; gq < 4; ++gq) {
            const float4 v = src[(i * 4 + gq) * 64];
            acc[i][4 * gq + 0] = v.x;
            acc[i][4 * gq + 1] = v.y;
            acc[i][4 * gq + 2] = v.z;
            acc[i][4 * gq + 3] = v.w;
        }
    lt_layernorm(acc, red, gamma, beta, eps, out, M, wn, m0);
}

static int ln_tail_gemm(const bf16_t *X, const bf16_t *Wimg32, const float *bias, const bf16_t *res, const float *gamma,
                        const float *beta, float eps, bf16_t *out, int M, int K, hipStream_t st, bool xpacked, float *img) {
    if (K % (16 * LT_PF) != 0) return fail(TSIM_EUNSUPPORTED, "ln_tail_gemm: K=%d", K);
    const int nb = (M + 31) / 32;
    const int S = !img || nb > LS_MAX_BLOCKS ? 1 : nb <= 64 ? 4 : nb <= 128 ? 2 : 1;
    if (S == 1) {
        hipLaunchKernelGGL(ln_tail_gemm_kernel<LT_PF>, dim3((unsigned)nb), dim3(256), 0, st, X, Wimg32, bias, res, gamma, beta, eps,
                           out, M, K, xpacked ? 1 : 0);
        TSIM_HIP_CHECK(hipGetLastError());
        return TSIM_OK;
    }
    float4 *im = reinterpret_cast<float4 *>(img);
    if (S == 4)
        hipLaunchKernelGGL((ln_split_gemm_kernel<LT_PF, 4>), dim3((unsigned)(nb * 4)), dim3(64), 0, st, X, Wimg32, bias, res, im, M, K,
                           xpacked ? 1 : 0);
    else
        hipLaunchKernelGGL((ln_split_gemm_kernel<LT_PF, 2>), dim3((unsigned)(nb * 2)), dim3(128), 0, st, X, Wimg32, bias, res, im, M,
                           K, xpacked ? 1 : 0);
    TSIM_HIP_CHECK(hipGetLastError());
    hipLaunchKernelGGL(ln_split_finish_kernel, dim3((unsigned)nb), dim3(256), 0, st, im, gamma, beta, eps, out, M);
    TSIM_HIP_CHECK(hipGetLastError());
    return TSIM_OK;
}

template <int NW, int NST>
static int ln_rows_gemm(const bf16_t *X, const bf16_t *Wimg32, const float *bias, const bf16_t *res, const float *gamma,
                        const float *beta, float eps, bf16_t *out, int M, int K, hipStream_t st, bool xpacked) {
    constexpr int lds = NST * (NW * 32 * LR_BK * 2 + LR_WBYTES);
    static_assert(lds <= 160 * 1024, "LDS budget");
    auto kern = ln_rows_gemm_kernel<NW, NST>;
    static DevOnce lds_once;
    TSIM_MAX_LDS(lds_once, kern, lds);
    if (K % LR_BK != 0 || K < NST * LR_BK) return fail(TSIM_EUNSUPPORTED, "ln_rows_gemm: K=%d", K);
    hipLaunchKernelGGL(kern, dim3((unsigned)((M + NW * 32 - 1) / (NW * 32))), dim3(NW * 64), lds, st, X, Wimg32, bias, res, gamma,
                       beta, eps, out, M, K, xpacked ? 1 : 0);
    TSIM_HIP_CHECK(hipGetLastError());
    return TSIM_OK;
}

static bool use_packed_layout(int H, int F) {
    return H == 384 && (3 * H) % X2_BN == 0 && F % X2_BN == 0 && F <= 2048;
}

template <int EPI>
static int gemm_plain(const bf16_t *X, const bf16_t *W, const bf16_t *Wp, const float *bias, bf16_t *out, int M, int N,
                      int K, hipStream_t st) {
    if (K == 384 && N % XR_BN == 0) return gemm_xres2<EPI, false>(X, W, bias, out, M, N, st);
    if (K >= 768 && gemm_pp_supported(N, K))
        return gemm_pp(EPI == EPI_GELU ? PP_EPI_GELU : PP_EPI_BIAS, X, Wp ? Wp : W, Wp != nullptr, bias, out, M, N, K, st);
    if (N % 128 == 0)
        return launch_gemm<128, 128, 64, 2, 2, EPI>(X, W, bias, nullptr, nullptr, nullptr, 0.f, out, M, N, K, st);
    return launch_gemm<128, 64, 64, 2, 2, EPI>(X, W, bias, nullptr, nullptr, nullptr, 0.f, out, M, N, K, st);
}

static int gemm_res_ln(const bf16_t *X, const bf16_t *W, const bf16_t *Wp, const float *bias, const bf16_t *res,
                       const float *gamma, const float *beta, float eps, bf16_t *out, int M, int N, int K, float *ybuf,
                       hipStream_t st, const bf16_t *Wimg = nullptr, const bf16_t *Wimg32 = nullptr, bool xpacked = false,
                       float *lnimg = nullptr) {
    if (xpacked && N != 384) return fail(TSIM_EINVAL, "gemm_res_ln: the packed operand layout is a hidden-384 form");
    if (ybuf && N >= 512 && N % 256 == 0 && gemm_pp_supported(N, K)) {
        int rc = gemm_pp(PP_EPI_F32, X, Wp ? Wp : W, Wp != nullptr, bias, ybuf, M, N, K, st);
        if (rc) return rc;
        return res_ln_rows(ybuf, res, gamma, beta, eps, out, nullptr, nullptr, M, N, st);
    }
    switch (N) {
        case 384: {
            bool after_rows = false;
            if (Wimg32) {
                const int t256 = M / 256;
                const int use = (t256 % 256) >= 128 ? t256 : (t256 / 256) * 256;
                if (use > 0) {
                    int rc = ln_rows_gemm<8, 3>(X, Wimg32, bias, res, gamma, beta, eps, out, use * 256, K, st, xpacked);
                    const int m1 = use * 256;
                    if (rc || m1 == M) return rc;
                    X += (int64_t)m1 * K; res += (int64_t)m1 * N; out += (int64_t)m1 * N; M -= m1;
                    after_rows = true;
                }
                if (M <= LS_MAX_BLOCKS * 32 && K % (16 * LT_PF) == 0)
                    return ln_tail_gemm(X, Wimg32, bias, res, gamma, beta, eps, out, M, K, st, xpacked, lnimg);
            }
            const int mt = (M + 127) / 128, full = (mt / 256) * 256, rem = mt - full;
            auto main_launch = [&](int rows) {
                return launch_gemm<128, 384, 64, 2, 4, EPI_RES_LN>(X, W, bias, res, gamma, beta, eps, out, rows, N, K, st, Wimg, xpacked);
            };
            if (rem > 0 && rem <= 96 && (full > 0 || after_rows)) {
                const int m_main = full * 128;
                if (full > 0) {
                    int rc = main_launch(m_main);
                    if (rc) return rc;
                }
                return launch_gemm<64, 384, 64, 2, 4, EPI_RES_LN>(X + (int64_t)m_main * K, W, bias, res + (int64_t)m_main * N,
                                                                  gamma, beta, eps, out + (int64_t)m_main * N, M - m_main, N, K, st, Wimg, xpacked);
            }
            return main_launch(M);
        }
        case 768: return launch_gemm<64, 768, 32, 1, 8, EPI_RES_LN>(X, W, bias, res, gamma, beta, eps, out, M, N, K, st);
        case 64: return launch_gemm<128, 64, 64, 4, 2, EPI_RES_LN>(X, W, bias, res, gamma, beta, eps, out, M, N, K, st);
        default: return fail(TSIM_EUNSUPPORTED, "encoder: hidden size %d has no fused LayerNorm GEMM (64, 384, 768)", N);
    }
}

}

extern "C" int tsim_encoder_create(const tsim_encoder_config *cfg, const tsim_encoder_weights_host *w,
                                   tsim_encoder **out) {
    TSIM_REQUIRE(cfg && w && out, "encoder_create: null pointer");
    const int H = cfg->hidden, F = cfg->ffn, L = cfg->num_layers;
    TSIM_REQUIRE(H == 64 || H == 384 || H == 768 || H == 1024, "encoder_create: hidden=%d unsupported (64, 384, 768, 1024)", H);
    TSIM_REQUIRE(cfg->heads > 0 && H % cfg->heads == 0, "encoder_create: heads=%d does not divide hidden=%d", cfg->heads, H);
    const int dh = H / cfg->heads;
    TSIM_REQUIRE(dh == 16 || dh == 32 || dh == 64, "encoder_create: head_dim=%d unsupported (16, 32, 64)", dh);
    TSIM_REQUIRE(F % 64 == 0 && L > 0 && cfg->max_tokens > 0 && cfg->max_seqs > 0, "encoder_create: bad ffn/layers/capacity");
    TSIM_REQUIRE(cfg->arch == TSIM_ARCH_BERT || cfg->arch == TSIM_ARCH_MPNET || cfg->arch == TSIM_ARCH_ROBERTA, "encoder_create: unknown arch");
    TSIM_REQUIRE(w->word_emb && w->pos_emb && w->emb_ln_g && w->emb_ln_b && w->layers, "encoder_create: missing weights");
    TSIM_REQUIRE(cfg->arch != TSIM_ARCH_MPNET || w->rel_bias, "encoder_create: MPNet needs rel_bias");
    const bool mx = cfg->weight_dtype == TSIM_W_MXFP8;
    TSIM_REQUIRE(cfg->weight_dtype == TSIM_W_BF16 || mx, "encoder_create: unknown weight_dtype %d", cfg->weight_dtype);
    if (mx && !(gemm_pp_mx_supported(H, H) && gemm_pp_mx_supported(3 * H, H) && gemm_pp_mx_supported(F, H) && gemm_pp_mx_supported(H, F)))
        return fail(TSIM_EUNSUPPORTED, "encoder_create: MXFP8 projections need hidden and ffn to be multiples of 256 (got %d, %d)", H, F);
    tsim_encoder *e = new tsim_encoder();
    e->cfg = *cfg;
    e->Tp = (cfg->max_tokens + 127) / 128 * 128 + 128;
    int rc = TSIM_OK;
    auto bail = [&](int code) {
        tsim_encoder_destroy(e);
        return code;
    };
    if ((rc = upload_f32(e, w->word_emb, (size_t)cfg->vocab * H, &e->word))) return bail(rc);
    if ((rc = upload_f32(e, w->pos_emb, (size_t)cfg->max_pos * H, &e->pos))) return bail(rc);
    if (w->type_emb && (rc = upload_f32(e, w->type_emb, H, &e->type0))) return bail(rc);
    if ((rc = upload_f32(e, w->emb_ln_g, H, &e->emb_g))) return bail(rc);
    if ((rc = upload_f32(e, w->emb_ln_b, H, &e->emb_b))) return bail(rc);
    if (cfg->arch == TSIM_ARCH_MPNET) {
        const int maxp = cfg->max_pos;
        e->relw = 2 * maxp - 1;
        std::vector<float> tab((size_t)cfg->heads * e->relw);
        for (int d = -(maxp - 1); d <= maxp - 1; ++d) {
            const int bk = mpnet_bucket(d, cfg->rel_buckets);
            for (int hh = 0; hh < cfg->heads; ++hh) tab[(size_t)hh * e->relw + d + maxp - 1] = w->rel_bias[bk * cfg->heads + hh];
        }
        if ((rc = upload_f32(e, tab.data(), tab.size(), &e->relb))) return bail(rc);
    }
    e->layers.resize(L);
    for (int l = 0; l < L; ++l) {
        const tsim_layer_weights_host &lw = w->layers[l];
        tsim_encoder::Layer &d = e->layers[l];
        if ((rc = upload_bf16(e, {lw.wq, lw.wk, lw.wv}, (size_t)H * H, &d.wqkv))) return bail(rc);
        if ((rc = upload_bf16(e, {lw.wo}, (size_t)H * H, &d.wo))) return bail(rc);
        if ((rc = upload_bf16(e, {lw.w1}, (size_t)F * H, &d.w1))) return bail(rc);
        if ((rc = upload_bf16(e, {lw.w2}, (size_t)H * F, &d.w2))) return bail(rc);
        if (mx) {
            if ((rc = upload_mxfp8(e, {lw.wq, lw.wk, lw.wv}, H, H, &d.qqkv, &d.sqkv))) return bail(rc);
            if ((rc = upload_mxfp8(e, {lw.wo}, H, H, &d.qo, &d.so))) return bail(rc);
            if ((rc = upload_mxfp8(e, {lw.w1}, F, H, &d.q1, &d.s1))) return bail(rc);
            if ((rc = upload_mxfp8(e, {lw.w2}, H, F, &d.q2, &d.s2))) return bail(rc);
        }
        auto repack = [&](const void *src, int n_rows, int kbytes, void **dst) {
            int r2 = dev_alloc(e, (size_t)n_rows * kbytes, dst);
            return r2 ? r2 : pack_w(src, *dst, n_rows, kbytes, gemm_pp_tile_width(n_rows), nullptr);
        };
        if (mx) {
            void *t;
            if ((rc = repack(d.qqkv, 3 * H, H, &t))) return bail(rc); d.qqkv = (uint8_t *)t;
            if ((rc = repack(d.qo, H, H, &t))) return bail(rc); d.qo = (uint8_t *)t;
            if ((rc = repack(d.q1, F, H, &t))) return bail(rc); d.q1 = (uint8_t *)t;
            if ((rc = repack(d.q2, H, F, &t))) return bail(rc); d.q2 = (uint8_t *)t;
        } else if (H >= 512 && H % 256 == 0 && gemm_pp_supported(H, H) && gemm_pp_supported(F, H) && gemm_pp_supported(H, F)) {
            if ((rc = repack(d.wqkv, 3 * H, H * 2, (void **)&d.pqkv))) return bail(rc);
            if ((rc = repack(d.wo, H, H * 2, (void **)&d.po))) return bail(rc);
        }
        if (!mx && H == 384 && F % 64 == 0) {
            if ((rc = dev_alloc(e, (size_t)H * H * 2, (void **)&d.lo))) return bail(rc);
            if ((rc = dev_alloc(e, (size_t)H * F * 2, (void **)&d.l2))) return bail(rc);
            hipLaunchKernelGGL(pack_gemm_w_kernel, dim3((unsigned)((H * H / 8 + 255) / 256)), dim3(256), 0, 0,
                               reinterpret_cast<const uint4 *>(d.wo), reinterpret_cast<uint4 *>(d.lo), 384, 64, H);
            hipLaunchKernelGGL(pack_gemm_w_kernel, dim3((unsigned)((H * F / 8 + 255) / 256)), dim3(256), 0, 0,
                               reinterpret_cast<const uint4 *>(d.w2), reinterpret_cast<uint4 *>(d.l2), 384, 64, F);
            if ((rc = dev_alloc(e, (size_t)H * H * 2, (void **)&d.lo32))) return bail(rc);
            if ((rc = dev_alloc(e, (size_t)H * F * 2, (void **)&d.l232))) return bail(rc);
            hipLaunchKernelGGL(pack_frag_w_kernel, dim3((unsigned)((H * H / 8 + 255) / 256)), dim3(256), 0, 0,
                               reinterpret_cast<const uint4 *>(d.wo), reinterpret_cast<uint4 *>(d.lo32), 384, H);
            hipLaunchKernelGGL(pack_frag_w_kernel, dim3((unsigned)((H * F / 8 + 255) / 256)), dim3(256), 0, 0,
                               reinterpret_cast<const uint4 *>(d.w2), reinterpret_cast<uint4 *>(d.l232), 384, F);
            if (hipGetLastError() != hipSuccess) return bail(fail(TSIM_EHIP, "LayerNorm GEMM weight packing failed"));
        }
        std::vector<float> bq(3 * (size_t)H);
        memcpy(bq.data(), lw.bq, H * 4);
        memcpy(bq.data() + H, lw.bk, H * 4);
        memcpy(bq.data() + 2 * H, lw.bv, H * 4);
        if ((rc = upload_f32(e, bq.data(), bq.size(), &d.bqkv))) return bail(rc);
        if ((rc = upload_f32(e, lw.bo, H, &d.bo))) return bail(rc);
        if ((rc = upload_f32(e, lw.b1, F, &d.b1))) return bail(rc);
        if ((rc = upload_f32(e, lw.b2, H, &d.b2))) return bail(rc);
        if ((rc = upload_f32(e, lw.ln1_g, H, &d.g1))) return bail(rc);
        if ((rc = upload_f32(e, lw.ln1_b, H, &d.be1))) return bail(rc);
        if ((rc = upload_f32(e, lw.ln2_g, H, &d.g2))) return bail(rc);
        if ((rc = upload_f32(e, lw.ln2_b, H, &d.be2))) return bail(rc);
    }
    const size_t Tp = e->Tp;
    struct { bf16_t **p; size_t n; } acts[] = {{&e->x0, Tp * H}, {&e->x1, Tp * H}, {&e->qkv, Tp * 3 * H},
                                               {&e->ctx, Tp * H}, {&e->h1, Tp * F}};
    for (auto &a : acts) {
        if ((rc = dev_alloc(e, a.n * 2, (void **)a.p))) return bail(rc);
        if (hipMemset(*a.p, 0, a.n * 2) != hipSuccess) return bail(fail(TSIM_EHIP, "hipMemset failed"));
    }
    if (H >= 512 && H % 256 == 0 && gemm_pp_supported(H, H)) {
        if ((rc = dev_alloc(e, Tp * H * 4, (void **)&e->ybuf))) return bail(rc);
        if (hipMemset(e->ybuf, 0, Tp * H * 4) != hipSuccess) return bail(fail(TSIM_EHIP, "hipMemset failed"));
    }
    if (!mx && H == 384 && F % 64 == 0) {
        const size_t blocks = (Tp + 31) / 32 < (size_t)LS_MAX_BLOCKS ? (Tp + 31) / 32 : (size_t)LS_MAX_BLOCKS;
        const size_t bytes = blocks * 4 * 12 * 64 * 16;
        if ((rc = dev_alloc(e, bytes, (void **)&e->lnimg))) return bail(rc);
        if (hipMemset(e->lnimg, 0, bytes) != hipSuccess) return bail(fail(TSIM_EHIP, "hipMemset failed"));
    }
    if ((size_t)cfg->max_seqs * H * 4 > Tp * 3 * H * 2 && (rc = dev_alloc(e, (size_t)cfg->max_seqs * H * 4, (void **)&e->head_x)))
        return bail(rc);
    if (mx) {
        struct { uint8_t **p; size_t n; } qb[] = {{&e->aq, Tp * H}, {&e->as, Tp * H / 32}, {&e->hq, Tp * F}, {&e->hs, Tp * F / 32}};
        for (auto &a : qb) {
            if ((rc = dev_alloc(e, a.n, (void **)a.p))) return bail(rc);
            if (hipMemset(*a.p, 0, a.n) != hipSuccess) return bail(fail(TSIM_EHIP, "hipMemset failed"));
        }
    }
    if ((rc = dev_alloc(e, 256, (void **)&e->err_flags))) return bail(rc);
    if (hipMemset(e->err_flags, 0, 256) != hipSuccess) return bail(fail(TSIM_EHIP, "hipMemset failed"));
    if (hipDeviceSynchronize() != hipSuccess) return bail(fail(TSIM_EHIP, "sync after upload failed"));
    *out = e;
    return TSIM_OK;
}

extern "C" int tsim_encoder_error_flags(tsim_encoder *e, int32_t *flags_host, void *stream) {
    TSIM_REQUIRE(e && flags_host, "encoder_error_flags: null pointer");
    hipStream_t st = reinterpret_cast<hipStream_t>(stream);
    TSIM_HIP_CHECK(hipMemcpyAsync(flags_host, e->err_flags, 4, hipMemcpyDeviceToHost, st));
    TSIM_HIP_CHECK(hipMemsetAsync(e->err_flags, 0, 4, st));
    TSIM_HIP_CHECK(hipStreamSynchronize(st));
    return TSIM_OK;
}

extern "C" int tsim_quantize_mxfp8(const void *x_bf16, int64_t rows, int K, void *q_out, void *scale_out, void *stream) {
    TSIM_REQUIRE(x_bf16 && q_out && scale_out, "quantize_mxfp8: null pointer");
    TSIM_REQUIRE(rows >= 0 && K > 0, "quantize_mxfp8: bad shape rows=%lld K=%d", (long long)rows, K);
    return quant_mx(static_cast<const bf16_t *>(x_bf16), rows, K, static_cast<uint8_t *>(q_out),
                    static_cast<uint8_t *>(scale_out), reinterpret_cast<hipStream_t>(stream));
}

extern "C" int tsim_gemm_mxfp8(const void *xq, const void *xs, const void *wq, const void *ws, const float *bias,
                               float *out_f32, int M, int N, int K, void *stream) {
    TSIM_REQUIRE(xq && xs && wq && ws && bias && out_f32, "gemm_mxfp8: null pointer");
    TSIM_REQUIRE(M >= 0 && N > 0 && K > 0, "gemm_mxfp8: bad shape M=%d N=%d K=%d", M, N, K);
    return gemm_pp_mx(PP_EPI_F32, static_cast<const uint8_t *>(xq), static_cast<const uint8_t *>(xs),
                      static_cast<const uint8_t *>(wq), 0, static_cast<const uint8_t *>(ws), bias, out_f32, nullptr, M, N, K,
                      reinterpret_cast<hipStream_t>(stream));
}

#ifdef TSIM_PP_STAMPS
extern "C" int tsim_debug_xr_stamps(unsigned long long *out8, int reset) {
    if (hipMemcpyFromSymbol(out8, HIP_SYMBOL(tsim::g_xr_stamps), 64) != hipSuccess) return 1;
    if (reset) { unsigned long long z[8] = {0}; if (hipMemcpyToSymbol(HIP_SYMBOL(tsim::g_xr_stamps), z, 64) != hipSuccess) return 1; }
    return 0;
}
#endif

extern "C" void tsim_encoder_destroy(tsim_encoder *e) {
    if (!e) return;
    for (void *p : e->allocs) (void)hipFree(p);
    delete e;
}

extern "C" int tsim_encoder_set_token_types(tsim_encoder *e, const float *type_emb_host, int32_t n_types) {
    TSIM_REQUIRE(e && type_emb_host, "encoder_set_token_types: null pointer");
    TSIM_REQUIRE(e->cfg.arch != TSIM_ARCH_MPNET, "encoder_set_token_types: BERT only (MPNet has no token-type table)");
    TSIM_REQUIRE(n_types >= 1, "encoder_set_token_types: n_types=%d < 1", n_types);
    float *tab = nullptr;
    if (int rc = upload_f32(e, type_emb_host, (size_t)n_types * e->cfg.hidden, &tab)) return rc;
    e->type0 = tab;
    e->n_types = n_types;
    return TSIM_OK;
}

extern "C" int tsim_encoder_set_cls_head(tsim_encoder *e, const float *pool_w_host, const float *pool_b_host,
                                         const float *cls_w_host, const float *cls_b_host, int32_t num_labels) {
    return tsim_encoder_set_cls_head_act(e, pool_w_host, pool_b_host, cls_w_host, cls_b_host, num_labels, TSIM_ACT_TANH);
}

extern "C" int tsim_encoder_set_cls_head_act(tsim_encoder *e, const float *pool_w_host, const float *pool_b_host,
                                             const float *cls_w_host, const float *cls_b_host, int32_t num_labels, int32_t act) {
    TSIM_REQUIRE(e && pool_w_host && pool_b_host && cls_w_host && cls_b_host, "encoder_set_cls_head: null pointer");
    TSIM_REQUIRE(e->cfg.arch != TSIM_ARCH_MPNET, "encoder_set_cls_head: BERT only");
    TSIM_REQUIRE(act == TSIM_ACT_TANH || act == TSIM_ACT_RELU, "encoder_set_cls_head: activation %d (TSIM_ACT_TANH, TSIM_ACT_RELU)", act);
    TSIM_REQUIRE(num_labels >= 1 && num_labels <= CLS_MAX_LABELS, "encoder_set_cls_head: num_labels=%d outside [1, %d]", num_labels,
                 CLS_MAX_LABELS);
    const int H = e->cfg.hidden;
    TSIM_REQUIRE(H % 64 == 0 && H <= CLS_WIDE_H, "encoder_set_cls_head: hidden=%d unsupported", H);
    std::vector<float> wT((size_t)H * H);
    for (int o = 0; o < H; ++o)
        for (int k = 0; k < H; ++k) wT[(size_t)k * H + o] = pool_w_host[(size_t)o * H + k];
    int rc;
    if ((rc = upload_f32(e, wT.data(), wT.size(), &e->head_wpT))) return rc;
    if ((rc = upload_f32(e, pool_b_host, H, &e->head_bp))) return rc;
    if ((rc = upload_f32(e, cls_w_host, (size_t)num_labels * H, &e->head_wc))) return rc;
    if ((rc = upload_f32(e, cls_b_host, num_labels, &e->head_bc))) return rc;
    e->n_labels = num_labels;
    e->head_act = act;
    return TSIM_OK;
}

extern "C" int tsim_encoder_forward(tsim_encoder *e, const int32_t *tok_ids, const int32_t *tok_pos,
                                    const int32_t *tok_col, const int32_t *cu_seqlens, int32_t T, int32_t B,
                                    int32_t max_len, float *pooled_f32, void *unit_bf16, int ld_unit, float *unit_rho_max,
                                    void *last_hidden_bf16, void *stream) {
    return tsim_encoder_forward_ex(e, tok_ids, nullptr, tok_pos, tok_col, cu_seqlens, T, B, max_len, pooled_f32, unit_bf16, ld_unit,
                                   unit_rho_max, last_hidden_bf16, nullptr, stream);
}

extern "C" int tsim_encoder_forward_ex(tsim_encoder *e, const int32_t *tok_ids, const int32_t *tok_type, const int32_t *tok_pos,
                                       const int32_t *tok_col, const int32_t *cu_seqlens, int32_t T, int32_t B,
                                       int32_t max_len, float *pooled_f32, void *unit_bf16, int ld_unit, float *unit_rho_max,
                                       void *last_hidden_bf16, float *logits_f32, void *stream) {
    TSIM_REQUIRE(e && cu_seqlens && (T == 0 || (tok_ids && tok_pos)), "encoder_forward: null pointer");
    TSIM_REQUIRE(!tok_type || e->n_types > 0, "encoder_forward: tok_type given but no token-type table was set "
                 "(tsim_encoder_set_token_types)");
    TSIM_REQUIRE(!logits_f32 || e->n_labels > 0, "encoder_forward: logits requested but no classification head was set "
                 "(tsim_encoder_set_cls_head)");
    TSIM_REQUIRE(T >= 0 && B >= 0 && T <= e->cfg.max_tokens && B <= e->cfg.max_seqs,
                 "encoder_forward: T=%d B=%d exceed capacity (%d tokens, %d sequences)", T, B, e->cfg.max_tokens, e->cfg.max_seqs);
    const int pos_span = max_len + (e->cfg.arch != TSIM_ARCH_BERT ? e->cfg.pad_id + 1 : 0);
    TSIM_REQUIRE(max_len >= 0 && pos_span <= e->cfg.max_pos,
                 "encoder_forward: sequences of %d tokens need position rows up to %d, the table has %d", max_len, pos_span - 1,
                 e->cfg.max_pos);
    TSIM_REQUIRE(!unit_bf16 || ld_unit >= e->cfg.hidden, "encoder_forward: ld_unit < hidden");
    TSIM_REQUIRE(!unit_bf16 || e->cfg.hidden <= 768, "encoder_forward: unit rows need a width <= 768 (got %d)", e->cfg.hidden);
    if (B == 0) return TSIM_OK;
    hipStream_t st = reinterpret_cast<hipStream_t>(stream);
    const tsim_encoder_config &c = e->cfg;
    const int H = c.hidden, F = c.ffn, dh = H / c.heads;
    const bool mx = c.weight_dtype == TSIM_W_MXFP8;
    int rc;
    if (T > 0) {
        const unsigned g = (unsigned)((T + 3) / 4);
        const int32_t *colp = tok_col ? tok_col : tok_pos;
        const int col_limit = tok_col || c.arch == TSIM_ARCH_BERT ? max_len : c.max_pos;
#define EMBED(V) hipLaunchKernelGGL(embed_ln_kernel<V>, dim3(g), dim3(256), 0, st, tok_ids, tok_pos, e->word, e->pos, e->type0, e->emb_g, e->emb_b, c.ln_eps, T, H, e->x0, c.vocab, c.max_pos, colp, col_limit, e->err_flags, nullptr, 0)
#define EMBED_T(V) hipLaunchKernelGGL((embed_ln_kernel<V, true>), dim3(g), dim3(256), 0, st, tok_ids, tok_pos, e->word, e->pos, e->type0, e->emb_g, e->emb_b, c.ln_eps, T, H, e->x0, c.vocab, c.max_pos, colp, col_limit, e->err_flags, tok_type, e->n_types)
        if (tok_type) {
            if (H == 64) EMBED_T(1); else if (H == 384) EMBED_T(6); else if (H == 768) EMBED_T(12); else EMBED_T(16);
        } else if (H == 64) EMBED(1); else if (H == 384) EMBED(6); else if (H == 768) EMBED(12); else EMBED(16);
#undef EMBED_T
#undef EMBED
        TSIM_HIP_CHECK(hipGetLastError());
        const float scale = 1.0f / sqrtf((float)dh);
        const bool rel = c.arch == TSIM_ARCH_MPNET;
        const bool pk = !mx && !rel && use_packed_layout(H, F);
        const int32_t *col = rel ? (tok_col ? tok_col : tok_pos) : nullptr;
        const int qblocks = (max_len + 31) / 32 > 0 ? (max_len + 31) / 32 : 1;
        const dim3 agrid((unsigned)(((B + 7) / 8) * 8), (unsigned)((c.heads + 3) / 4), (unsigned)qblocks);
        for (int l = 0; l < c.num_layers; ++l) {
            const tsim_encoder::Layer &L = e->layers[l];
            if (mx) {
                if (l == 0 && (rc = quant_mx(e->x0, T, H, e->aq, e->as, st))) return rc;
                if ((rc = gemm_pp_mx(PP_EPI_BIAS, e->aq, e->as, L.qqkv, 1, L.sqkv, L.bqkv, e->qkv, nullptr, T, 3 * H, H, st))) return rc;
            } else if (pk) {
                if ((rc = gemm_xres2<EPI_BIAS, true>(e->x0, L.wqkv, L.bqkv, e->qkv, T, 3 * H, st))) return rc;
            } else if ((rc = gemm_plain<EPI_BIAS>(e->x0, L.wqkv, L.pqkv, L.bqkv, e->qkv, T, 3 * H, H, st))) return rc;
#define ATT(D)                                                                                                 \
    do {                                                                                                       \
        if (rel)                                                                                               \
            hipLaunchKernelGGL((attention_kernel<D, true>), agrid, dim3(256), 0, st, e->qkv, cu_seqlens, col,  \
                               e->relb, e->relw, H, c.heads, scale, e->ctx, B, 1);                                         \
        else if (pk)                                                                                           \
            hipLaunchKernelGGL((attention_kernel<D, false, true>), agrid, dim3(256), 0, st, e->qkv, cu_seqlens, col, \
                               e->relb, e->relw, H, c.heads, scale, e->ctx, B, 1);                                         \
        else                                                                                                   \
            hipLaunchKernelGGL((attention_kernel<D, false>), agrid, dim3(256), 0, st, e->qkv, cu_seqlens, col, \
                               e->relb, e->relw, H, c.heads, scale, e->ctx, B, 1);                                         \
    } while (0)
            if (dh == 16) ATT(16); else if (dh == 32) ATT(32); else ATT(64);
#undef ATT
            TSIM_HIP_CHECK(hipGetLastError());
            if (mx) {
                if ((rc = quant_mx(e->ctx, T, H, e->aq, e->as, st))) return rc;
                if ((rc = gemm_pp_mx(PP_EPI_F32, e->aq, e->as, L.qo, 1, L.so, L.bo, e->ybuf, nullptr, T, H, H, st))) return rc;
                if ((rc = res_ln_rows(e->ybuf, e->x0, L.g1, L.be1, c.ln_eps, e->x1, e->aq, e->as, T, H, st))) return rc;
                if ((rc = gemm_pp_mx(PP_EPI_GELU_MX, e->aq, e->as, L.q1, 1, L.s1, L.b1, e->hq, e->hs, T, F, H, st))) return rc;
                if ((rc = gemm_pp_mx(PP_EPI_F32, e->hq, e->hs, L.q2, 1, L.s2, L.b2, e->ybuf, nullptr, T, H, F, st))) return rc;
                if ((rc = res_ln_rows(e->ybuf, e->x1, L.g2, L.be2, c.ln_eps, e->x0, e->aq, e->as, T, H, st))) return rc;
                continue;
            }
            if ((rc = gemm_res_ln(e->ctx, L.wo, L.po, L.bo, e->x0, L.g1, L.be1, c.ln_eps, e->x1, T, H, H, e->ybuf, st, L.lo, L.lo32, false, e->lnimg))) return rc;
            if (pk) {
                if ((rc = gemm_xres2<EPI_GELU, true>(e->x1, L.w1, L.b1, e->h1, T, F, st))) return rc;
            } else if ((rc = gemm_plain<EPI_GELU>(e->x1, L.w1, nullptr, L.b1, e->h1, T, F, H, st))) return rc;
            if ((rc = gemm_res_ln(e->h1, L.w2, nullptr, L.b2, e->x1, L.g2, L.be2, c.ln_eps, e->x0, T, H, F, e->ybuf, st, L.l2, L.l232, pk, e->lnimg))) return rc;
        }
        if (last_hidden_bf16)
            TSIM_HIP_CHECK(hipMemcpyAsync(last_hidden_bf16, e->x0, (size_t)T * H * 2, hipMemcpyDeviceToDevice, st));
    }
    if (pooled_f32 || unit_bf16) {
        const unsigned g = (unsigned)((B + 3) / 4);
#define POOL(V) hipLaunchKernelGGL(pool_packed_kernel<V>, dim3(g), dim3(256), 0, st, e->x0, cu_seqlens, B, H, pooled_f32, (unit_t *)unit_bf16, ld_unit, unit_bf16 ? unit_rho_max : nullptr)
        if (H % 8 != 0 || H > 1024 || (unit_bf16 && ld_unit % 8 != 0))
            return fail(TSIM_EUNSUPPORTED, "encoder: pooling needs a hidden size that is a multiple of 8, at most 1024 (got %d)", H);
        if (((uintptr_t)pooled_f32 | (uintptr_t)unit_bf16) & 15)
            return fail(TSIM_EINVAL, "encoder: pooled / unit outputs must be 16-byte aligned");
        if (H <= 512) POOL(1); else POOL(2);
#undef POOL
        TSIM_HIP_CHECK(hipGetLastError());
    }
    if (logits_f32) {
        const dim3 cgrid((unsigned)((B + CLS_ROWS - 1) / CLS_ROWS)), cblock((unsigned)H);
#define CLS_WIDE(MAXH, ACT)                                                                                       \
    hipLaunchKernelGGL((cls_head_wide_kernel<MAXH, ACT>), cgrid, cblock, 0, st, e->x0, cu_seqlens, B, H, e->head_wpT, \
                       e->head_bp, e->head_wc, e->head_bc, e->n_labels, logits_f32)
        if (e->head_act == TSIM_ACT_RELU) {
            if (H <= CLS_MAX_H) CLS_WIDE(CLS_MAX_H, TSIM_ACT_RELU); else CLS_WIDE(CLS_WIDE_H, TSIM_ACT_RELU);
        } else if (H <= CLS_MAX_H) {
            hipLaunchKernelGGL(cls_head_kernel, cgrid, cblock, 0, st, e->x0, cu_seqlens,
                               B, H, e->head_wpT, e->head_bp, e->head_wc, e->head_bc, e->n_labels, logits_f32);
        } else CLS_WIDE(CLS_WIDE_H, TSIM_ACT_TANH);
#undef CLS_WIDE
        TSIM_HIP_CHECK(hipGetLastError());
    }
    return TSIM_OK;
}

extern "C" int tsim_encoder_forward_head(tsim_encoder *e, const int32_t *tok_ids, const int32_t *tok_type, const int32_t *tok_pos,
                                         const int32_t *tok_col, const int32_t *cu_seqlens, int32_t T, int32_t B, int32_t max_len,
                                         const tsim_sentence_head *head, float *emb_f32, void *unit_f16, int ld_unit,
                                         float *unit_rho_max, void *last_hidden_bf16, void *stream) {
    if (!head)
        return tsim_encoder_forward_ex(e, tok_ids, tok_type, tok_pos, tok_col, cu_seqlens, T, B, max_len, emb_f32, unit_f16, ld_unit,
                                       unit_rho_max, last_hidden_bf16, nullptr, stream);
    TSIM_REQUIRE(e, "encoder_forward_head: null encoder");
    const int H = e->cfg.hidden, mode = head->pool_mode, d_out = head->d_out;
    TSIM_REQUIRE(mode >= TSIM_POOL_MEAN && mode <= TSIM_POOL_MEAN_SQRT_LEN, "encoder_forward_head: unknown pool_mode %d", mode);
    TSIM_REQUIRE(head->normalize == 0 || head->normalize == 1, "encoder_forward_head: normalize=%d is not 0 / 1", head->normalize);
    TSIM_REQUIRE(d_out >= 0, "encoder_forward_head: d_out=%d < 0", d_out);
    if (d_out) {
        TSIM_REQUIRE(head->dense_w, "encoder_forward_head: d_out=%d without dense_w", d_out);
        if (int rc = dense_check(H, d_out, head->dense_act, head->dense_w)) return rc;
    } else {
        TSIM_REQUIRE(!head->dense_w && !head->dense_b, "encoder_forward_head: dense weights given with d_out = 0");
    }
    const int width = d_out ? d_out : H;
    TSIM_REQUIRE(!unit_f16 || width <= 768, "encoder_forward_head: unit rows need a final width <= 768 (got %d)", width);
    TSIM_REQUIRE(!unit_f16 || (ld_unit >= width && ld_unit % 8 == 0), "encoder_forward_head: ld_unit=%d (final width %d)", ld_unit,
                 width);
    TSIM_REQUIRE(H % 8 == 0 && H <= 1024, "encoder_forward_head: pooling needs hidden %% 8 == 0 and <= 1024 (got %d)", H);
    TSIM_REQUIRE((((uintptr_t)emb_f32 | (uintptr_t)unit_f16) & 15) == 0, "encoder_forward_head: outputs must be 16-byte aligned");
    if (int rc = tsim_encoder_forward_ex(e, tok_ids, tok_type, tok_pos, tok_col, cu_seqlens, T, B, max_len, nullptr, nullptr, 0,
                                         nullptr, last_hidden_bf16, nullptr, stream))
        return rc;
    if (B == 0 || (!emb_f32 && !unit_f16)) return TSIM_OK;
    hipStream_t st = reinterpret_cast<hipStream_t>(stream);
    float *px = d_out ? (e->head_x ? e->head_x : reinterpret_cast<float *>(e->qkv)) : emb_f32;
    unit_t *pu = d_out ? nullptr : static_cast<unit_t *>(unit_f16);
    const bool norm = !d_out && head->normalize;
    const unsigned g = (unsigned)((B + 3) / 4);
#define POOL(NP, M, N) hipLaunchKernelGGL((pool_packed_kernel<NP, M, N>), dim3(g), dim3(256), 0, st, e->x0, cu_seqlens, B, H, px, pu, ld_unit, pu ? unit_rho_max : nullptr)
#define POOL_NP(M, N) do { if (H <= 512) POOL(1, M, N); else POOL(2, M, N); } while (0)
#define POOL_M(N) do { switch (mode) { case TSIM_POOL_MEAN: POOL_NP(TSIM_POOL_MEAN, N); break; case TSIM_POOL_CLS: POOL_NP(TSIM_POOL_CLS, N); break; \
                                       case TSIM_POOL_MAX: POOL_NP(TSIM_POOL_MAX, N); break; default: POOL_NP(TSIM_POOL_MEAN_SQRT_LEN, N); } } while (0)
    if (norm) POOL_M(true); else POOL_M(false);
#undef POOL_M
#undef POOL_NP
#undef POOL
    TSIM_HIP_CHECK(hipGetLastError());
    if (d_out)
        return dense_rows_launch(px, B, H, head->dense_w, head->dense_b, d_out, head->dense_act, head->normalize, emb_f32,
                                 static_cast<unit_t *>(unit_f16), ld_unit, unit_f16 ? unit_rho_max : nullptr, st);
    return TSIM_OK;
}

extern "C" int tsim_dense_rows(const float *x, int64_t B, int d_in, const float *w, const float *b, int d_out, int act, int normalize,
                               float *out, void *stream) {
    TSIM_REQUIRE(x && out, "dense_rows: null pointer");
    TSIM_REQUIRE(B >= 0 && B <= INT32_MAX - DN_ROWS, "dense_rows: bad row count %lld", (long long)B);
    TSIM_REQUIRE(normalize == 0 || normalize == 1, "dense_rows: normalize=%d is not 0 / 1", normalize);
    if (int rc = dense_check(d_in, d_out, act, w)) return rc;
    TSIM_REQUIRE((((uintptr_t)x | (uintptr_t)out) & 15) == 0, "dense_rows: x and out must be 16-byte aligned");
    return dense_rows_launch(x, (int)B, d_in, w, b, d_out, act, normalize, out, nullptr, 0, nullptr, reinterpret_cast<hipStream_t>(stream));
}

#include "span_pool.h"
```

Baseline: 831,000.

## Keep hidden-state activations in packed tile layout between encoder layers

Adds a group_off helper and respacked/opacked flags so the residual+LayerNorm epilogues can read residuals and write outputs in the 32-row packed layout. The QKV and FFN-up xres2 GEMMs gain a packed-X template path, which lets x0/x1 stay packed between layers instead of row-major. The goal is better-coalesced and more cache-friendly operand loads in the downstream GEMMs. The trade-off is more strided epilogue stores and extra layout bookkeeping, and the last layer must still write row-major for pooling. Timing stamp slots are also extended for profiling.

```diff
diff --git a/text_similarity_amd/csrc/encoder.hip b/text_similarity_amd/csrc/encoder.hip
--- a/text_similarity_amd/csrc/encoder.hip
+++ b/text_similarity_amd/csrc/encoder.hip
@@ -16,6 +16,9 @@
 
 __device__ __forceinline__ int64_t packed_off(int64_t t, int f, int W) {
     return ((t >> 5) * (W >> 3) + (f >> 3)) * 256 + (t & 31) * 8 + (f & 7);
+}
+__device__ __forceinline__ int64_t group_off(int64_t t, int g, int W, int packed) {
+    return packed ? packed_off(t, 8 * g, W) * 2 : (t * W + 8 * g) * 2;
 }
 
 template <int VPL, bool TYPED = false>
@@ -92,7 +95,8 @@
 __global__ __launch_bounds__(WAVES_M *WAVES_N * 64) void gemm_bf16_kernel(
     const bf16_t *__restrict__ X, const bf16_t *__restrict__ W, const float *__restrict__ bias,
     const bf16_t *__restrict__ res, const float *__restrict__ gamma, const float *__restrict__ beta, float eps,
-    bf16_t *__restrict__ out, int M, int N, int K, int mtiles, int ntiles, const bf16_t *__restrict__ Wimg, int xpacked) {
+    bf16_t *__restrict__ out, int M, int N, int K, int mtiles, int ntiles, const bf16_t *__restrict__ Wimg, int xpacked,
+    int respacked, int opacked) {
     constexpr int NW = WAVES_M * WAVES_N;
     constexpr int TM = BM / WAVES_M, TN = BN / WAVES_N, MT = TM / 32, NT = TN / 32;
     constexpr int RB = BK * 2;
@@ -254,15 +258,18 @@
     if constexpr (EPI == EPI_RES_LN) {
         float *red = reinterpret_cast<float *>(smem);
         __builtin_amdgcn_s_barrier();
+        const int g0 = (n0 + wn * TN) / 8 + h;
+        const int rgs = (int)group_off(0, 1, N, respacked), ogs = (int)group_off(0, 1, N, opacked);
 #pragma unroll
         for (int j = 0; j < MT; ++j) {
             const int64_t m = m0 + wm * TM + j * 32 + r;
             const int64_t mr = m < M ? m : M - 1;
+            const char *rp = reinterpret_cast<const char *>(res) + group_off(mr, g0, N, respacked);
 #pragma unroll
             for (int i = 0; i < NT; ++i)
 #pragma unroll
                 for (int gq = 0; gq < 4; gq += 2) {
-                    const uint4 o = *reinterpret_cast<const uint4 *>(res + mr * N + n0 + wn * TN + i * 32 + 8 * gq + 8 * h);
+                    const uint4 o = *reinterpret_cast<const uint4 *>(rp + (i * 4 + gq) * rgs);
                     auto s0 = __builtin_amdgcn_permlane32_swap(o.x, o.z, false, false);
                     auto s1 = __builtin_amdgcn_permlane32_swap(o.y, o.w, false, false);
                     const uint32_t a0 = s0[0], c0 = s0[1], a1 = s1[0], c1 = s1[1];
@@ -329,13 +336,12 @@
                     pk[2 * gq + 1] = pack_bf16x2(y2, y3);
                 }
                 const int64_t m = m0 + wm * TM + j * 32 + r;
+                char *op = reinterpret_cast<char *>(out) + group_off(m, g0, N, opacked);
 #pragma unroll
                 for (int gq = 0; gq < 4; gq += 2) {
                     auto s0 = __builtin_amdgcn_permlane32_swap(pk[2 * gq], pk[2 * gq + 2], false, false);
                     auto s1 = __builtin_amdgcn_permlane32_swap(pk[2 * gq + 1], pk[2 * gq + 3], false, false);
-                    if (m < M)
-                        *reinterpret_cast<uint4 *>(out + m * N + n0 + wn * TN + i * 32 + 8 * gq + 8 * h) =
-                            make_uint4(s0[0], s1[0], s0[1], s1[1]);
+                    if (m < M) *reinterpret_cast<uint4 *>(op + (i * 4 + gq) * ogs) = make_uint4(s0[0], s1[0], s0[1], s1[1]);
                 }
             }
         }
@@ -367,12 +373,12 @@
 typedef __attribute__((ext_vector_type(4))) uint32_t u32x4;
 
 #ifdef TSIM_PP_STAMPS
-__device__ unsigned long long g_xr_stamps[8];
+__device__ unsigned long long g_xr_stamps[16];
 #define XR_T() __builtin_amdgcn_s_memtime()
 #ifndef TSIM_XR_STAMP_TID
 #define TSIM_XR_STAMP_TID 0
 #endif
-#define XR_ACC(i, v) do { if (threadIdx.x == TSIM_XR_STAMP_TID) atomicAdd(&g_xr_stamps[i], (unsigned long long)(v)); } while (0)
+#define XR_ACC(i, v) do { if (threadIdx.x == TSIM_XR_STAMP_TID) atomicAdd(&g_xr_stamps[(i) + (EPI == EPI_GELU ? 8 : 0)], (unsigned long long)(v)); } while (0)
 #else
 #define XR_T() 0ull
 #define XR_ACC(i, v) do { } while (0)
@@ -385,7 +391,7 @@
 
 constexpr int X2_BN = 96, X2_BK = 128, X2_NSTAGE = 6, X2_PD = 4, X2_KG = 3, X2_NSUB = 3;
 
-template <int EPI, bool PK>
+template <int EPI, bool PK, bool XPK>
 __global__ __launch_bounds__(512) void gemm_xres2_kernel(const bf16_t *__restrict__ X, const bf16_t *__restrict__ W,
                                                          const float *__restrict__ bias, bf16_t *__restrict__ out,
                                                          int M, int N, int items_total) {
@@ -467,18 +473,23 @@
 
 #pragma unroll
     for (int i = 0; i < X2_PD; ++i) issue(i, i);
-    [[maybe_unused]] unsigned x2_n = 0, x2_w = 0, x2_c = 0, x2_e = 0;
+    [[maybe_unused]] unsigned x2_n = 0, x2_w = 0, x2_c = 0, x2_e = 0, x2_r = 0, x2_nr = 0;
     auto run_item = [&](f32x16 (&cur)[X2_NSUB], f32x16 (&old)[X2_NSUB], int item, auto with_old) __attribute__((always_inline)) {
         constexpr bool OLD = decltype(with_old)::value;
         if (item / ntiles != cur_mb) {
+            [[maybe_unused]] const unsigned long long xr0 = XR_T();
             cur_mb = item / ntiles;
             m0 = cur_mb * BMX + wave * 32;
-            const bf16_t *xp = X + (int64_t)(m0 + r) * K + 8 * h;
-#pragma unroll
-            for (int s = 0; s < KSTEPS; ++s) bx[s] = *reinterpret_cast<const bf16x8 *>(xp + 16 * s);
+            const char *xp = reinterpret_cast<const char *>(X) + group_off(m0 + r, h, K, XPK);
+            constexpr int xgs = XPK ? 512 : 16;
+#pragma unroll
+            for (int s = 0; s < KSTEPS; ++s) bx[s] = *reinterpret_cast<const bf16x8 *>(xp + 2 * s * xgs);
 #pragma unroll
             for (int s = 0; s < KSTEPS; ++s) asm volatile("" : "+v"(bx[s]));
             young1 = young2 = young3 = 0;
+#ifdef TSIM_PP_STAMPS
+            x2_r += (unsigned)(XR_T() - xr0); x2_nr += 1;
+#endif
         }
         const int n0 = (item % ntiles) * X2_BN;
         const uint32_t baddr = bias_lds + (n0 + 4 * h) * 4;
@@ -581,7 +592,7 @@
         }
     };
     if (lastA) flush(accA); else flush(accB);
-    XR_ACC(0, x2_n); XR_ACC(1, x2_w); XR_ACC(3, x2_c); XR_ACC(4, x2_e); XR_ACC(6, x2_n / 3);
+    XR_ACC(0, x2_n); XR_ACC(1, x2_w); XR_ACC(3, x2_c); XR_ACC(4, x2_e); XR_ACC(6, x2_n / 3); XR_ACC(2, 1); XR_ACC(5, x2_r); XR_ACC(7, x2_nr);
 }
 
 __global__ __launch_bounds__(256) void pack_gemm_w_kernel(const uint4 *__restrict__ W, uint4 *__restrict__ img, int BN, int BK, int K) {
@@ -607,7 +618,8 @@
 __global__ __launch_bounds__(NW * 64) void ln_rows_gemm_kernel(const bf16_t *__restrict__ X, const bf16_t *__restrict__ Wimg,
                                                                const float *__restrict__ bias, const bf16_t *__restrict__ res,
                                                                const float *__restrict__ gamma, const float *__restrict__ beta,
-                                                               float eps, bf16_t *__restrict__ out, int M, int K, int xpacked) {
+                                                               float eps, bf16_t *__restrict__ out, int M, int K, int xpacked,
+                                                               int respacked, int opacked) {
     constexpr int N = 384, XBYTES = NW * 32 * LR_BK * 2, STAGE = XBYTES + LR_WBYTES;
     constexpr int XP = XBYTES / 1024, PIECES = STAGE / 1024, PPW = PIECES / NW;
     static_assert(PIECES % NW == 0 && XP == 2 * NW, "every wave issues two X pieces and PPW - 2 W pieces per k-tile");
@@ -701,11 +713,12 @@
     const int64_t m = m0 + wave * 32 + r;
     const bool live = m < M;
     const int64_t mr = live ? m : M - 1;
+    const uint32_t ro = (uint32_t)group_off(mr, h, N, respacked), rgs = (uint32_t)group_off(0, 1, N, respacked);
 #pragma unroll
     for (int t = 0; t < 12; ++t)
 #pragma unroll
         for (int gq = 0; gq < 4; gq += 2) {
-            const uint4 o = *reinterpret_cast<const uint4 *>(res + mr * N + 32 * t + 8 * gq + 8 * h);
+            const uint4 o = *reinterpret_cast<const uint4 *>(reinterpret_cast<const char *>(res) + (ro + (4 * t + gq) * rgs));
             auto s0 = __builtin_amdgcn_permlane32_swap(o.x, o.z, false, false);
             auto s1 = __builtin_amdgcn_permlane32_swap(o.y, o.w, false, false);
             const uint32_t a0 = s0[0], c0 = s0[1], a1 = s1[0], c1 = s1[1];
@@ -744,6 +757,7 @@
         else
             rstd = 1.0f / sqrtf(tot / (float)N + eps);
     }
+    const uint32_t oo = (uint32_t)group_off(m, h, N, opacked), ogs = (uint32_t)group_off(0, 1, N, opacked);
 #pragma unroll
     for (int t = 0; t < 12; ++t) {
         uint32_t pk[8];
@@ -762,7 +776,8 @@
         for (int gq = 0; gq < 4; gq += 2) {
             auto s0 = __builtin_amdgcn_permlane32_swap(pk[2 * gq], pk[2 * gq + 2], false, false);
             auto s1w = __builtin_amdgcn_permlane32_swap(pk[2 * gq + 1], pk[2 * gq + 3], false, false);
-            if (live) *reinterpret_cast<uint4 *>(out + m * N + 32 * t + 8 * gq + 8 * h) = make_uint4(s0[0], s1w[0], s0[1], s1w[1]);
+            if (live)
+                *reinterpret_cast<uint4 *>(reinterpret_cast<char *>(out) + (oo + (4 * t + gq) * ogs)) = make_uint4(s0[0], s1w[0], s0[1], s1w[1]);
         }
     }
 }
@@ -1441,7 +1456,7 @@
 template <int BM, int BN, int BK, int WM, int WN, int EPI, int NST = 2>
 static int launch_gemm(const bf16_t *X, const bf16_t *W, const float *bias, const bf16_t *res, const float *gamma,
                        const float *beta, float eps, bf16_t *out, int M, int N, int K, hipStream_t st,
-                       const bf16_t *Wimg = nullptr, bool xpacked = false) {
+                       const bf16_t *Wimg = nullptr, bool xpacked = false, bool respacked = false, bool opacked = false) {
     constexpr int lds = gemm_lds_bytes<BM, BN, BK, WM, WN, NST>();
     static_assert(lds <= 160 * 1024, "LDS budget");
     auto kern = gemm_bf16_kernel<BM, BN, BK, WM, WN, EPI, NST>;
@@ -1452,17 +1467,17 @@
     const int grid = ((mtiles + 7) / 8) * 8 * ntiles;
     if (Wimg && ntiles != 1) return fail(TSIM_EINVAL, "gemm: a packed W image needs BN == N");
     hipLaunchKernelGGL(kern, dim3(grid), dim3(WM * WN * 64), lds, st, X, W, bias, res, gamma, beta, eps, out, M, N, K,
-                       mtiles, ntiles, Wimg, xpacked ? 1 : 0);
+                       mtiles, ntiles, Wimg, xpacked ? 1 : 0, respacked ? 1 : 0, opacked ? 1 : 0);
     TSIM_HIP_CHECK(hipGetLastError());
     return TSIM_OK;
 }
 
-template <int EPI, bool PK>
+template <int EPI, bool PK, bool XPK = false>
 static int gemm_xres2(const bf16_t *X, const bf16_t *W, const float *bias, bf16_t *out, int M, int N, hipStream_t st) {
     constexpr int lds = X2_NSTAGE * X2_BN * X2_BK * 2 + 8192;
     if (N > 2048) return fail(TSIM_EUNSUPPORTED, "gemm_xres2: N=%d > 2048", N);
     if (((int64_t)M + 256) * N * 2 >= (1ll << 32)) return fail(TSIM_EUNSUPPORTED, "gemm_xres2: output of %d x %d exceeds 4 GiB", M, N);
-    auto kern = gemm_xres2_kernel<EPI, PK>;
+    auto kern = gemm_xres2_kernel<EPI, PK, XPK>;
     static DevOnce lds_once;
     TSIM_MAX_LDS(lds_once, kern, lds);
     const int items = ((M + 255) / 256) * (N / X2_BN);
@@ -1478,7 +1493,7 @@
 template <int PF>
 __device__ __forceinline__ void lt_gemm_slice(const bf16_t *__restrict__ X, const bf16_t *__restrict__ Wimg32,
                                               const float *__restrict__ bias, const bf16_t *__restrict__ res, int M, int K,
-                                              int xpacked, int wn, int m0, f32x16 (&acc)[3]) {
+                                              int xpacked, int respacked, int wn, int m0, f32x16 (&acc)[3]) {
     constexpr int N = 384, NT = 3;
     const int lane = threadIdx.x & 63;
     const int r = lane & 31, h = lane >> 5;
@@ -1536,11 +1551,12 @@
     {
         const int64_t m = m0 + r;
         const int64_t mr = m < M ? m : M - 1;
+        const uint32_t ro = (uint32_t)group_off(mr, wn * 12 + h, N, respacked), rgs = (uint32_t)group_off(0, 1, N, respacked);
 #pragma unroll
         for (int i = 0; i < NT; ++i)
 #pragma unroll
             for (int gq = 0; gq < 4; gq += 2) {
-                const uint4 o = *reinterpret_cast<const uint4 *>(res + mr * N + wn * 96 + i * 32 + 8 * gq + 8 * h);
+                const uint4 o = *reinterpret_cast<const uint4 *>(reinterpret_cast<const char *>(res) + (ro + (4 * i + gq) * rgs));
                 auto s0 = __builtin_amdgcn_permlane32_swap(o.x, o.z, false, false);
                 auto s1 = __builtin_amdgcn_permlane32_swap(o.y, o.w, false, false);
                 const uint32_t a0 = s0[0], c0 = s0[1], a1 = s1[0], c1 = s1[1];
@@ -1558,7 +1574,7 @@
 
 __device__ __forceinline__ void lt_layernorm(f32x16 (&acc)[3], float *red, const float *__restrict__ gamma,
                                              const float *__restrict__ beta, float eps, bf16_t *__restrict__ out, int M, int wn,
-                                             int m0) {
+                                             int m0, int opacked) {
     constexpr int N = 384, NT = 3, WAVES_N = 4, BM = 32;
     const int lane = threadIdx.x & 63;
     const int r = lane & 31, h = lane >> 5;
@@ -1608,12 +1624,13 @@
             pk[2 * gq + 1] = pack_bf16x2(y2, y3);
         }
         const int64_t m = m0 + r;
+        const uint32_t oo = (uint32_t)group_off(m, wn * 12 + h, N, opacked), ogs = (uint32_t)group_off(0, 1, N, opacked);
 #pragma unroll
         for (int gq = 0; gq < 4; gq += 2) {
             auto s0 = __builtin_amdgcn_permlane32_swap(pk[2 * gq], pk[2 * gq + 2], false, false);
             auto s1 = __builtin_amdgcn_permlane32_swap(pk[2 * gq + 1], pk[2 * gq + 3], false, false);
             if (m < M)
-                *reinterpret_cast<uint4 *>(out + m * N + wn * 96 + i * 32 + 8 * gq + 8 * h) = make_uint4(s0[0], s1[0], s0[1], s1[1]);
+                *reinterpret_cast<uint4 *>(reinterpret_cast<char *>(out) + (oo + (4 * i + gq) * ogs)) = make_uint4(s0[0], s1[0], s0[1], s1[1]);
         }
     }
 }
@@ -1621,13 +1638,14 @@
 template <int PF>
 __global__ __launch_bounds__(256) __attribute__((amdgpu_waves_per_eu(1, 1))) void ln_tail_gemm_kernel(
     const bf16_t *__restrict__ X, const bf16_t *__restrict__ Wimg32, const float *__restrict__ bias, const bf16_t *__restrict__ res,
-    const float *__restrict__ gamma, const float *__restrict__ beta, float eps, bf16_t *__restrict__ out, int M, int K, int xpacked) {
+    const float *__restrict__ gamma, const float *__restrict__ beta, float eps, bf16_t *__restrict__ out, int M, int K, int xpacked,
+    int respacked, int opacked) {
     __shared__ float red[2 * 4 * 32];
     const int wn = __builtin_amdgcn_readfirstlane(threadIdx.x >> 6);
     const int m0 = blockIdx.x * 32;
     f32x16 acc[3];
-    lt_gemm_slice<PF>(X, Wimg32, bias, res, M, K, xpacked, wn, m0, acc);
-    lt_layernorm(acc, red, gamma, beta, eps, out, M, wn, m0);
+    lt_gemm_slice<PF>(X, Wimg32, bias, res, M, K, xpacked, respacked, wn, m0, acc);
+    lt_layernorm(acc, red, gamma, beta, eps, out, M, wn, m0, opacked);
 }
 
 constexpr int LS_MAX_BLOCKS = 256;
@@ -1635,12 +1653,12 @@
 template <int PF, int S>
 __global__ __launch_bounds__(256 / S) __attribute__((amdgpu_waves_per_eu(1, 1))) void ln_split_gemm_kernel(
     const bf16_t *__restrict__ X, const bf16_t *__restrict__ Wimg32, const float *__restrict__ bias, const bf16_t *__restrict__ res,
-    float4 *__restrict__ img, int M, int K, int xpacked) {
+    float4 *__restrict__ img, int M, int K, int xpacked, int respacked) {
     const int blk = blockIdx.x / S, sl = blockIdx.x % S;
     const int wn = __builtin_amdgcn_readfirstlane(sl * (4 / S) + (threadIdx.x >> 6));
     const int m0 = blk * 32;
     f32x16 acc[3];
-    lt_gemm_slice<PF>(X, Wimg32, bias, res, M, K, xpacked, wn, m0, acc);
+    lt_gemm_slice<PF>(X, Wimg32, bias, res, M, K, xpacked, respacked, wn, m0, acc);
     float4 *dst = img + (int64_t)(blk * 4 + wn) * 12 * 64 + (threadIdx.x & 63);
 #pragma unroll
     for (int i = 0; i < 3; ++i)
@@ -1651,7 +1669,7 @@
 
 __global__ __launch_bounds__(256) void ln_split_finish_kernel(const float4 *__restrict__ img, const float *__restrict__ gamma,
                                                               const float *__restrict__ beta, float eps, bf16_t *__restrict__ out,
-                                                              int M) {
+                                                              int M, int opacked) {
     __shared__ float red[2 * 4 * 32];
     const int wn = __builtin_amdgcn_readfirstlane(threadIdx.x >> 6);
     const int m0 = blockIdx.x * 32;
@@ -1667,44 +1685,47 @@
             acc[i][4 * gq + 2] = v.z;
             acc[i][4 * gq + 3] = v.w;
         }
-    lt_layernorm(acc, red, gamma, beta, eps, out, M, wn, m0);
+    lt_layernorm(acc, red, gamma, beta, eps, out, M, wn, m0, opacked);
 }
 
 static int ln_tail_gemm(const bf16_t *X, const bf16_t *Wimg32, const float *bias, const bf16_t *res, const float *gamma,
-                        const float *beta, float eps, bf16_t *out, int M, int K, hipStream_t st, bool xpacked, float *img) {
+                        const float *beta, float eps, bf16_t *out, int M, int K, hipStream_t st, bool xpacked, float *img, bool respacked,
+                        bool opacked) {
+    const int rpk = respacked ? 1 : 0, opk = opacked ? 1 : 0;
     if (K % (16 * LT_PF) != 0) return fail(TSIM_EUNSUPPORTED, "ln_tail_gemm: K=%d", K);
     const int nb = (M + 31) / 32;
     const int S = !img || nb > LS_MAX_BLOCKS ? 1 : nb <= 64 ? 4 : nb <= 128 ? 2 : 1;
     if (S == 1) {
         hipLaunchKernelGGL(ln_tail_gemm_kernel<LT_PF>, dim3((unsigned)nb), dim3(256), 0, st, X, Wimg32, bias, res, gamma, beta, eps,
-                           out, M, K, xpacked ? 1 : 0);
+                           out, M, K, xpacked ? 1 : 0, rpk, opk);
         TSIM_HIP_CHECK(hipGetLastError());
         return TSIM_OK;
     }
     float4 *im = reinterpret_cast<float4 *>(img);
     if (S == 4)
         hipLaunchKernelGGL((ln_split_gemm_kernel<LT_PF, 4>), dim3((unsigned)(nb * 4)), dim3(64), 0, st, X, Wimg32, bias, res, im, M, K,
-                           xpacked ? 1 : 0);
+                           xpacked ? 1 : 0, rpk);
     else
         hipLaunchKernelGGL((ln_split_gemm_kernel<LT_PF, 2>), dim3((unsigned)(nb * 2)), dim3(128), 0, st, X, Wimg32, bias, res, im, M,
-                           K, xpacked ? 1 : 0);
+                           K, xpacked ? 1 : 0, rpk);
     TSIM_HIP_CHECK(hipGetLastError());
-    hipLaunchKernelGGL(ln_split_finish_kernel, dim3((unsigned)nb), dim3(256), 0, st, im, gamma, beta, eps, out, M);
+    hipLaunchKernelGGL(ln_split_finish_kernel, dim3((unsigned)nb), dim3(256), 0, st, im, gamma, beta, eps, out, M, opk);
     TSIM_HIP_CHECK(hipGetLastError());
     return TSIM_OK;
 }
 
 template <int NW, int NST>
 static int ln_rows_gemm(const bf16_t *X, const bf16_t *Wimg32, const float *bias, const bf16_t *res, const float *gamma,
-                        const float *beta, float eps, bf16_t *out, int M, int K, hipStream_t st, bool xpacked) {
+                        const float *beta, float eps, bf16_t *out, int M, int K, hipStream_t st, bool xpacked, bool respacked, bool opacked) {
     constexpr int lds = NST * (NW * 32 * LR_BK * 2 + LR_WBYTES);
     static_assert(lds <= 160 * 1024, "LDS budget");
     auto kern = ln_rows_gemm_kernel<NW, NST>;
     static DevOnce lds_once;
     TSIM_MAX_LDS(lds_once, kern, lds);
     if (K % LR_BK != 0 || K < NST * LR_BK) return fail(TSIM_EUNSUPPORTED, "ln_rows_gemm: K=%d", K);
+    if (((int64_t)M + 256) * 768 >= (1ll << 32)) return fail(TSIM_EUNSUPPORTED, "ln_rows_gemm: %d rows of 384 exceed 4 GiB", M);
     hipLaunchKernelGGL(kern, dim3((unsigned)((M + NW * 32 - 1) / (NW * 32))), dim3(NW * 64), lds, st, X, Wimg32, bias, res, gamma,
-                       beta, eps, out, M, K, xpacked ? 1 : 0);
+                       beta, eps, out, M, K, xpacked ? 1 : 0, respacked ? 1 : 0, opacked ? 1 : 0);
     TSIM_HIP_CHECK(hipGetLastError());
     return TSIM_OK;
 }
@@ -1727,8 +1748,8 @@
 static int gemm_res_ln(const bf16_t *X, const bf16_t *W, const bf16_t *Wp, const float *bias, const bf16_t *res,
                        const float *gamma, const float *beta, float eps, bf16_t *out, int M, int N, int K, float *ybuf,
                        hipStream_t st, const bf16_t *Wimg = nullptr, const bf16_t *Wimg32 = nullptr, bool xpacked = false,
-                       float *lnimg = nullptr) {
-    if (xpacked && N != 384) return fail(TSIM_EINVAL, "gemm_res_ln: the packed operand layout is a hidden-384 form");
+                       float *lnimg = nullptr, bool respacked = false, bool opacked = false) {
+    if ((xpacked || respacked || opacked) && N != 384) return fail(TSIM_EINVAL, "gemm_res_ln: the packed layouts are a hidden-384 form");
     if (ybuf && N >= 512 && N % 256 == 0 && gemm_pp_supported(N, K)) {
         int rc = gemm_pp(PP_EPI_F32, X, Wp ? Wp : W, Wp != nullptr, bias, ybuf, M, N, K, st);
         if (rc) return rc;
@@ -1741,18 +1762,18 @@
                 const int t256 = M / 256;
                 const int use = (t256 % 256) >= 128 ? t256 : (t256 / 256) * 256;
                 if (use > 0) {
-                    int rc = ln_rows_gemm<8, 3>(X, Wimg32, bias, res, gamma, beta, eps, out, use * 256, K, st, xpacked);
+                    int rc = ln_rows_gemm<8, 3>(X, Wimg32, bias, res, gamma, beta, eps, out, use * 256, K, st, xpacked, respacked, opacked);
                     const int m1 = use * 256;
                     if (rc || m1 == M) return rc;
                     X += (int64_t)m1 * K; res += (int64_t)m1 * N; out += (int64_t)m1 * N; M -= m1;
                     after_rows = true;
                 }
                 if (M <= LS_MAX_BLOCKS * 32 && K % (16 * LT_PF) == 0)
-                    return ln_tail_gemm(X, Wimg32, bias, res, gamma, beta, eps, out, M, K, st, xpacked, lnimg);
+                    return ln_tail_gemm(X, Wimg32, bias, res, gamma, beta, eps, out, M, K, st, xpacked, lnimg, respacked, opacked);
             }
             const int mt = (M + 127) / 128, full = (mt / 256) * 256, rem = mt - full;
             auto main_launch = [&](int rows) {
-                return launch_gemm<128, 384, 64, 2, 4, EPI_RES_LN>(X, W, bias, res, gamma, beta, eps, out, rows, N, K, st, Wimg, xpacked);
+                return launch_gemm<128, 384, 64, 2, 4, EPI_RES_LN>(X, W, bias, res, gamma, beta, eps, out, rows, N, K, st, Wimg, xpacked, respacked, opacked);
             };
             if (rem > 0 && rem <= 96 && (full > 0 || after_rows)) {
                 const int m_main = full * 128;
@@ -1761,7 +1782,7 @@
                     if (rc) return rc;
                 }
                 return launch_gemm<64, 384, 64, 2, 4, EPI_RES_LN>(X + (int64_t)m_main * K, W, bias, res + (int64_t)m_main * N,
-                                                                  gamma, beta, eps, out + (int64_t)m_main * N, M - m_main, N, K, st, Wimg, xpacked);
+                                                                  gamma, beta, eps, out + (int64_t)m_main * N, M - m_main, N, K, st, Wimg, xpacked, respacked, opacked);
             }
             return main_launch(M);
         }
@@ -1927,9 +1948,9 @@
 }
 
 #ifdef TSIM_PP_STAMPS
-extern "C" int tsim_debug_xr_stamps(unsigned long long *out8, int reset) {
-    if (hipMemcpyFromSymbol(out8, HIP_SYMBOL(tsim::g_xr_stamps), 64) != hipSuccess) return 1;
-    if (reset) { unsigned long long z[8] = {0}; if (hipMemcpyToSymbol(HIP_SYMBOL(tsim::g_xr_stamps), z, 64) != hipSuccess) return 1; }
+extern "C" int tsim_debug_xr_stamps(unsigned long long *out16, int reset) {
+    if (hipMemcpyFromSymbol(out16, HIP_SYMBOL(tsim::g_xr_stamps), 128) != hipSuccess) return 1;
+    if (reset) { unsigned long long z[16] = {0}; if (hipMemcpyToSymbol(HIP_SYMBOL(tsim::g_xr_stamps), z, 128) != hipSuccess) return 1; }
     return 0;
 }
 #endif
@@ -2029,11 +2050,14 @@
         const dim3 agrid((unsigned)(((B + 7) / 8) * 8), (unsigned)((c.heads + 3) / 4), (unsigned)qblocks);
         for (int l = 0; l < c.num_layers; ++l) {
             const tsim_encoder::Layer &L = e->layers[l];
+            const bool x0pk = pk && l > 0, x0pk_next = pk && l + 1 < c.num_layers;
             if (mx) {
                 if (l == 0 && (rc = quant_mx(e->x0, T, H, e->aq, e->as, st))) return rc;
                 if ((rc = gemm_pp_mx(PP_EPI_BIAS, e->aq, e->as, L.qqkv, 1, L.sqkv, L.bqkv, e->qkv, nullptr, T, 3 * H, H, st))) return rc;
             } else if (pk) {
-                if ((rc = gemm_xres2<EPI_BIAS, true>(e->x0, L.wqkv, L.bqkv, e->qkv, T, 3 * H, st))) return rc;
+                rc = x0pk ? gemm_xres2<EPI_BIAS, true, true>(e->x0, L.wqkv, L.bqkv, e->qkv, T, 3 * H, st)
+                          : gemm_xres2<EPI_BIAS, true>(e->x0, L.wqkv, L.bqkv, e->qkv, T, 3 * H, st);
+                if (rc) return rc;
             } else if ((rc = gemm_plain<EPI_BIAS>(e->x0, L.wqkv, L.pqkv, L.bqkv, e->qkv, T, 3 * H, H, st))) return rc;
 #define ATT(D)                                                                                                 \
     do {                                                                                                       \
@@ -2059,11 +2083,11 @@
                 if ((rc = res_ln_rows(e->ybuf, e->x1, L.g2, L.be2, c.ln_eps, e->x0, e->aq, e->as, T, H, st))) return rc;
                 continue;
             }
-            if ((rc = gemm_res_ln(e->ctx, L.wo, L.po, L.bo, e->x0, L.g1, L.be1, c.ln_eps, e->x1, T, H, H, e->ybuf, st, L.lo, L.lo32, false, e->lnimg))) return rc;
+            if ((rc = gemm_res_ln(e->ctx, L.wo, L.po, L.bo, e->x0, L.g1, L.be1, c.ln_eps, e->x1, T, H, H, e->ybuf, st, L.lo, L.lo32, false, e->lnimg, x0pk, pk))) return rc;
             if (pk) {
-                if ((rc = gemm_xres2<EPI_GELU, true>(e->x1, L.w1, L.b1, e->h1, T, F, st))) return rc;
+                if ((rc = gemm_xres2<EPI_GELU, true, true>(e->x1, L.w1, L.b1, e->h1, T, F, st))) return rc;
             } else if ((rc = gemm_plain<EPI_GELU>(e->x1, L.w1, nullptr, L.b1, e->h1, T, F, H, st))) return rc;
-            if ((rc = gemm_res_ln(e->h1, L.w2, nullptr, L.b2, e->x1, L.g2, L.be2, c.ln_eps, e->x0, T, H, F, e->ybuf, st, L.l2, L.l232, pk, e->lnimg))) return rc;
+            if ((rc = gemm_res_ln(e->h1, L.w2, nullptr, L.b2, e->x1, L.g2, L.be2, c.ln_eps, e->x0, T, H, F, e->ybuf, st, L.l2, L.l232, pk, e->lnimg, pk, x0pk_next))) return rc;
         }
         if (last_hidden_bf16)
             TSIM_HIP_CHECK(hipMemcpyAsync(last_hidden_bf16, e->x0, (size_t)T * H * 2, hipMemcpyDeviceToDevice, st));
```

After: 845,700 (median of 6 runs). 1.8% higher.
